# AIBluefisher/DReg-NeRF

Hardware: AMD Instinct MI355X
Metric: nerf_pairs_per_sec_regtr_fwd_bwd_128 (higher is better)
Workload: dtype bf16; 1 GPU; RegTR fwd+bwd+AdamW, shell-R synthetic pairs, 128^3 grids, 4 pairs (8 grids) per GPU per step, random-init weights; global_batch_pairs=4, resolution=128, fpn_head=active-set (identical results; rows around occupied voxels), parallelism=dp1

## Files before the change

### dreg_nerf_amd/csrc/common.h

```cpp
#pragma once
#include <hip/hip_runtime.h>
#include <stdint.h>

#define DREG_OK 0
#define DREG_EINVAL (-1)
#define DREG_ELAUNCH (-2)

typedef uint16_t bf16_t;
typedef __attribute__((ext_vector_type(8))) short bf16x8_t;
typedef __attribute__((ext_vector_type(4))) short bf16x4_t;
typedef __attribute__((ext_vector_type(4))) float f32x4_t;
typedef __attribute__((ext_vector_type(16))) float f32x16_t;

__device__ __forceinline__ float bf2f(bf16_t h) { return __uint_as_float(((uint32_t)h) << 16); }
typedef __attribute__((__vector_size__(2 * sizeof(__bf16)))) __bf16 hw_bf16x2_t;
typedef __attribute__((__vector_size__(2 * sizeof(float)))) float hw_f32x2_t;
__device__ __forceinline__ bf16_t f2bf(float f) { return __builtin_bit_cast(unsigned short, (__bf16)f); }
__device__ __forceinline__ uint32_t f2bf2(float lo, float hi) {
    const hw_f32x2_t v = {lo, hi};
    return __builtin_bit_cast(uint32_t, __builtin_convertvector(v, hw_bf16x2_t));
}

template <typename T> struct Elem;
template <> struct Elem<float> {
    static __device__ __forceinline__ float ld(const float* p) { return *p; }
    static __device__ __forceinline__ void st(float* p, float v) { *p = v; }
};
template <> struct Elem<bf16_t> {
    static __device__ __forceinline__ float ld(const bf16_t* p) { return bf2f(*p); }
    static __device__ __forceinline__ void st(bf16_t* p, float v) { *p = f2bf(v); }
};

__device__ __forceinline__ uint32_t fdiv(uint32_t n, uint32_t magic) {
    return magic ? __umulhi(n, magic) : n;
}
static inline uint32_t host_magic(uint32_t d) {
    return d <= 1 ? 0u : (uint32_t)((0x100000000ull + d - 1) / d);
}

__device__ __forceinline__ float wave_sum(float v) {
#pragma unroll
    for (int o = 32; o > 0; o >>= 1) v += __shfl_xor(v, o, 64);
    return v;
}
__device__ __forceinline__ float wave_max(float v) {
#pragma unroll
    for (int o = 32; o > 0; o >>= 1) v = fmaxf(v, __shfl_xor(v, o, 64));
    return v;
}

#ifdef DREG_PROBE
#define DREG_KNOB(type, name, value) static type name = value
#else
#define DREG_KNOB(type, name, value) static constexpr type name = value
#endif

#define DREG_LAUNCH_CHECK()                                   \
    do {                                                      \
        hipError_t e__ = hipGetLastError();                   \
        if (e__ != hipSuccess) return (int)e__;               \
    } while (0)
```

### dreg_nerf_amd/csrc/pointset.hip

```cpp
#include "common.h"
#include <cstring>
#include <rocprim/device/device_radix_sort.hpp>
#include <rocprim/device/device_scan.hpp>

__device__ __forceinline__ void ld4(const float* p, float (&v)[4]) { const float4 q = *reinterpret_cast<const float4*>(p); v[0] = q.x; v[1] = q.y; v[2] = q.z; v[3] = q.w; }
__device__ __forceinline__ void ld4(const bf16_t* p, float (&v)[4]) {
    const uint2 q = *reinterpret_cast<const uint2*>(p);
    v[0] = __uint_as_float(q.x << 16); v[1] = __uint_as_float(q.x & 0xffff0000u); v[2] = __uint_as_float(q.y << 16); v[3] = __uint_as_float(q.y & 0xffff0000u);
}
__device__ __forceinline__ void st4(float* p, const float (&v)[4]) { *reinterpret_cast<float4*>(p) = make_float4(v[0], v[1], v[2], v[3]); }
__device__ __forceinline__ void st4(bf16_t* p, const float (&v)[4]) { *reinterpret_cast<uint2*>(p) = make_uint2(f2bf2(v[0], v[1]), f2bf2(v[2], v[3])); }
template <typename TO>
__global__ __launch_bounds__(256) void layernorm_fwd_kernel(const float* __restrict__ x, const float* __restrict__ g, const float* __restrict__ b,
                                                            const float* __restrict__ pe, TO* __restrict__ y, float* __restrict__ stats, int N, float eps)
{
    const int row = blockIdx.x * 4 + (threadIdx.x >> 6), lane = threadIdx.x & 63;
    if (row >= N) return;
    const float4 v = *reinterpret_cast<const float4*>(x + (size_t)row * 256 + lane * 4);
    const float mean = wave_sum(v.x + v.y + v.z + v.w) * (1.f / 256.f);
    const float d0 = v.x - mean, d1 = v.y - mean, d2 = v.z - mean, d3 = v.w - mean;
    const float var = wave_sum(d0 * d0 + d1 * d1 + d2 * d2 + d3 * d3) * (1.f / 256.f);
    const float rstd = 1.0f / sqrtf(var + eps);
    const float4 gg = *reinterpret_cast<const float4*>(g + lane * 4), bb = *reinterpret_cast<const float4*>(b + lane * 4);
    float o[4] = {d0 * rstd * gg.x + bb.x, d1 * rstd * gg.y + bb.y, d2 * rstd * gg.z + bb.z, d3 * rstd * gg.w + bb.w};
    if (pe) { const float4 p = *reinterpret_cast<const float4*>(pe + (size_t)row * 256 + lane * 4); o[0] += p.x; o[1] += p.y; o[2] += p.z; o[3] += p.w; }
    st4(y + (size_t)row * 256 + lane * 4, o);
    if (lane == 0) { stats[2 * row] = mean; stats[2 * row + 1] = rstd; }
}
__global__ __launch_bounds__(256) void layernorm_fwd2_kernel(const float* __restrict__ x, const float* __restrict__ g, const float* __restrict__ b,
                                                             const float* __restrict__ pe, int pe_rows, float* __restrict__ y32, bf16_t* __restrict__ y16,
                                                             float* __restrict__ stats, int N, float eps)
{
    const int row = blockIdx.x * 4 + (threadIdx.x >> 6), lane = threadIdx.x & 63;
    if (row >= N) return;
    const float4 v = *reinterpret_cast<const float4*>(x + (size_t)row * 256 + lane * 4);
    const float mean = wave_sum(v.x + v.y + v.z + v.w) * (1.f / 256.f);
    const float d0 = v.x - mean, d1 = v.y - mean, d2 = v.z - mean, d3 = v.w - mean;
    const float var = wave_sum(d0 * d0 + d1 * d1 + d2 * d2 + d3 * d3) * (1.f / 256.f);
    const float rstd = 1.0f / sqrtf(var + eps);
    const float4 gg = *reinterpret_cast<const float4*>(g + lane * 4), bb = *reinterpret_cast<const float4*>(b + lane * 4);
    float o[4] = {d0 * rstd * gg.x + bb.x, d1 * rstd * gg.y + bb.y, d2 * rstd * gg.z + bb.z, d3 * rstd * gg.w + bb.w};
    if (y32) st4(y32 + (size_t)row * 256 + lane * 4, o);
    if (y16) {
        if (pe) { const float4 p = *reinterpret_cast<const float4*>(pe + (size_t)(row % pe_rows) * 256 + lane * 4); o[0] += p.x; o[1] += p.y; o[2] += p.z; o[3] += p.w; }
        st4(y16 + (size_t)row * 256 + lane * 4, o);
    }
    if (lane == 0) { stats[2 * row] = mean; stats[2 * row + 1] = rstd; }
}
template <typename TG>
__global__ __launch_bounds__(256) void layernorm_bwd_kernel(const float* __restrict__ x, const TG* __restrict__ dy, const float* __restrict__ g,
                                                            const float* __restrict__ stats, float* __restrict__ dx, float* __restrict__ part,
                                                            int N, int rows_per_block, const float* dx_add, const float* dx_add2 = nullptr,
                                                            bf16_t* __restrict__ dx_bf = nullptr, const bf16_t* __restrict__ dy2 = nullptr)
{
    const int wave = threadIdx.x >> 6, lane = threadIdx.x & 63;
    const float4 gg = *reinterpret_cast<const float4*>(g + lane * 4);
    float dg[4] = {0, 0, 0, 0}, db[4] = {0, 0, 0, 0};
    const int r0 = blockIdx.x * rows_per_block;
    const int rend = min(r0 + rows_per_block, N);
    const float gv[4] = {gg.x, gg.y, gg.z, gg.w};
    for (int rb = r0 + wave; rb < rend; rb += 16) {
        constexpr int U = 4;
        float4 v[U], old[U], old2[U];
        float d[U][4], mean[U], rstd[U];
#pragma unroll
        for (int u = 0; u < U; ++u) {
            const int row = rb + 4 * u;
            if (row < rend) {
                v[u] = *reinterpret_cast<const float4*>(x + (size_t)row * 256 + lane * 4);
                ld4(dy + (size_t)row * 256 + lane * 4, d[u]);
                if (dy2) { float e2[4]; ld4(dy2 + (size_t)row * 256 + lane * 4, e2); d[u][0] += e2[0]; d[u][1] += e2[1]; d[u][2] += e2[2]; d[u][3] += e2[3]; }
                mean[u] = stats[2 * row]; rstd[u] = stats[2 * row + 1];
                if (dx_add) old[u] = *reinterpret_cast<const float4*>(dx_add + (size_t)row * 256 + lane * 4);
                if (dx_add2) old2[u] = *reinterpret_cast<const float4*>(dx_add2 + (size_t)row * 256 + lane * 4);
            }
        }
#pragma unroll
        for (int u = 0; u < U; ++u) {
            const int row = rb + 4 * u;
            if (row < rend) {
                const float xh[4] = {(v[u].x - mean[u]) * rstd[u], (v[u].y - mean[u]) * rstd[u], (v[u].z - mean[u]) * rstd[u], (v[u].w - mean[u]) * rstd[u]};
                float s1 = 0.f, s2 = 0.f;
#pragma unroll
                for (int i = 0; i < 4; ++i) { s1 += d[u][i] * gv[i]; s2 += d[u][i] * gv[i] * xh[i]; dg[i] += d[u][i] * xh[i]; db[i] += d[u][i]; }
                s1 = wave_sum(s1) * (1.f / 256.f); s2 = wave_sum(s2) * (1.f / 256.f);
                float o[4];
#pragma unroll
                for (int i = 0; i < 4; ++i) o[i] = rstd[u] * (d[u][i] * gv[i] - s1 - xh[i] * s2);
                if (dx_add) { o[0] += old[u].x; o[1] += old[u].y; o[2] += old[u].z; o[3] += old[u].w; }
                if (dx_add2) { o[0] += old2[u].x; o[1] += old2[u].y; o[2] += old2[u].z; o[3] += old2[u].w; }
                *reinterpret_cast<float4*>(dx + (size_t)row * 256 + lane * 4) = make_float4(o[0], o[1], o[2], o[3]);
                if (dx_bf) st4(dx_bf + (size_t)row * 256 + lane * 4, o);
            }
        }
    }
    __shared__ float red[4][512];
#pragma unroll
    for (int i = 0; i < 4; ++i) { red[wave][lane * 4 + i] = dg[i]; red[wave][256 + lane * 4 + i] = db[i]; }
    __syncthreads();
    for (int c = threadIdx.x; c < 512; c += 256) part[(size_t)blockIdx.x * 512 + c] = red[0][c] + red[1][c] + red[2][c] + red[3][c];
}
__global__ void layernorm_bwd_final_kernel(const float* __restrict__ part, float* __restrict__ dg, float* __restrict__ db, int nblk, int accumulate)
{
    const int c = blockIdx.x * (blockDim.x >> 6) + (threadIdx.x >> 6), lane = threadIdx.x & 63;
    if (c >= 512) return;
    double s = 0.0;
#pragma unroll 8
    for (int k = lane; k < nblk; k += 64) s += part[(size_t)k * 512 + c];
#pragma unroll
    for (int o = 32; o > 0; o >>= 1) s += __shfl_xor(s, o, 64);
    if (lane == 0) {
        float* dst = c < 256 ? dg + c : db + (c - 256);
        *dst = accumulate ? *dst + (float)s : (float)s;
    }
}

struct LnFinalDesc { const float* part; float* dg; float* db; int nblk, accumulate; };
static_assert(sizeof(LnFinalDesc) == 32, "LayerNorm final record: 32 bytes");
__global__ void layernorm_bwd_final_batched_kernel(const LnFinalDesc* __restrict__ descs)
{
    const LnFinalDesc d = descs[blockIdx.x >> 7];
    const int c = (blockIdx.x & 127) * (blockDim.x >> 6) + (threadIdx.x >> 6), lane = threadIdx.x & 63;
    if (c >= 512) return;
    double s = 0.0;
#pragma unroll 8
    for (int k = lane; k < d.nblk; k += 64) s += d.part[(size_t)k * 512 + c];
#pragma unroll
    for (int o = 32; o > 0; o >>= 1) s += __shfl_xor(s, o, 64);
    if (lane == 0) {
        float* dst = c < 256 ? d.dg + c : d.db + (c - 256);
        *dst = d.accumulate ? *dst + (float)s : (float)s;
    }
}

__global__ void posenc_sine_kernel(const float* __restrict__ xyz, float* __restrict__ pe, int N, float scale2pi, float log_temp)
{
    const size_t total = (size_t)N * 256;
    for (size_t i = blockIdx.x * (size_t)blockDim.x + threadIdx.x; i < total; i += (size_t)gridDim.x * blockDim.x) {
        const int c = (int)(i & 255), n = (int)(i >> 8);
        float v = 0.f;
        if (c < 252) {
            const int coord = c / 84, f = c - coord * 84;
            const float dim_t = powf(expf(log_temp), (float)(2 * (f >> 1)) / 84.f);
            const float arg = (xyz[(size_t)n * 3 + coord] * scale2pi) / dim_t;
            v = (f & 1) ? cosf(arg) : sinf(arg);
        }
        pe[i] = v;
    }
}

__global__ __launch_bounds__(256) void overlap_fwd_kernel(const float* __restrict__ f, const float* __restrict__ w, const float* __restrict__ b,
                                                          float* __restrict__ s, int N)
{
    const int row = blockIdx.x * 4 + (threadIdx.x >> 6), lane = threadIdx.x & 63;
    if (row >= N) return;
    const float4 v = *reinterpret_cast<const float4*>(f + (size_t)row * 256 + lane * 4);
    const float4 ww = *reinterpret_cast<const float4*>(w + lane * 4);
    const float z = wave_sum(v.x * ww.x + v.y * ww.y + v.z * ww.z + v.w * ww.w) + b[0];
    if (lane == 0) s[row] = 1.f / (1.f + expf(-z));
}
__global__ __launch_bounds__(256) void overlap_bwd_kernel(const float* __restrict__ f, const float* __restrict__ w, const float* __restrict__ s,
                                                          const float* __restrict__ gy, float* __restrict__ df, float* __restrict__ part,
                                                          int N, int rows_per_block, const float* df_add = nullptr)
{
    const int wave = threadIdx.x >> 6, lane = threadIdx.x & 63;
    const float4 ww = *reinterpret_cast<const float4*>(w + lane * 4);
    float dw[4] = {0, 0, 0, 0}, dbias = 0.f;
    const int r0 = blockIdx.x * rows_per_block;
    for (int row = r0 + wave; row < min(r0 + rows_per_block, N); row += 4) {
        const float sv = s[row], dl = gy[row] * sv * (1.f - sv);
        const float4 v = *reinterpret_cast<const float4*>(f + (size_t)row * 256 + lane * 4);
        float4 o = make_float4(dl * ww.x, dl * ww.y, dl * ww.z, dl * ww.w);
        if (df_add) {
            const float4 p = *reinterpret_cast<const float4*>(df_add + (size_t)row * 256 + lane * 4);
            o.x = p.x + o.x; o.y = p.y + o.y; o.z = p.z + o.z; o.w = p.w + o.w;
        }
        *reinterpret_cast<float4*>(df + (size_t)row * 256 + lane * 4) = o;
        dw[0] += dl * v.x; dw[1] += dl * v.y; dw[2] += dl * v.z; dw[3] += dl * v.w;
        dbias += dl;
    }
    __shared__ float red[4][257];
#pragma unroll
    for (int i = 0; i < 4; ++i) red[wave][lane * 4 + i] = dw[i];
    if (lane == 0) red[wave][256] = dbias;
    __syncthreads();
    for (int c = threadIdx.x; c < 257; c += 256) part[(size_t)blockIdx.x * 257 + c] = red[0][c] + red[1][c] + red[2][c] + red[3][c];
}
__global__ void overlap_bwd_final_kernel(const float* __restrict__ part, float* __restrict__ dw, float* __restrict__ db, int nblk, int accumulate = 0)
{
    const int c = blockIdx.x * (blockDim.x >> 6) + (threadIdx.x >> 6), lane = threadIdx.x & 63;
    if (c >= 257) return;
    double s = 0.0;
    for (int k = lane; k < nblk; k += 64) s += part[(size_t)k * 257 + c];
#pragma unroll
    for (int o = 32; o > 0; o >>= 1) s += __shfl_xor(s, o, 64);
    if (lane == 0) { float* dst = c < 256 ? dw + c : db; *dst = accumulate ? *dst + (float)s : (float)s; }
}

template <typename TY, typename TG, typename TO>
__global__ void relu_bwd_kernel(const TY* __restrict__ y, const TG* __restrict__ g, TO* __restrict__ out, size_t n)
{
    for (size_t i = blockIdx.x * (size_t)blockDim.x + threadIdx.x; i < n; i += (size_t)gridDim.x * blockDim.x)
        Elem<TO>::st(out + i, Elem<TY>::ld(y + i) > 0.f ? Elem<TG>::ld(g + i) : 0.f);
}

__device__ void jacobi_eig3(double A[3][3], double V[3][3])
{
    for (int i = 0; i < 3; ++i) for (int j = 0; j < 3; ++j) V[i][j] = (i == j);
    for (int sweep = 0; sweep < 30; ++sweep) {
        const double off = fabs(A[0][1]) + fabs(A[0][2]) + fabs(A[1][2]);
        if (off < 1e-300) break;
        for (int p = 0; p < 2; ++p)
            for (int q = p + 1; q < 3; ++q) {
                if (fabs(A[p][q]) < 1e-300) continue;
                const double theta = (A[q][q] - A[p][p]) / (2.0 * A[p][q]);
                const double t = (theta >= 0 ? 1.0 : -1.0) / (fabs(theta) + sqrt(theta * theta + 1.0));
                const double c = 1.0 / sqrt(t * t + 1.0), s = t * c;
                for (int k = 0; k < 3; ++k) { const double akp = A[k][p], akq = A[k][q]; A[k][p] = c * akp - s * akq; A[k][q] = s * akp + c * akq; }
                for (int k = 0; k < 3; ++k) { const double apk = A[p][k], aqk = A[q][k]; A[p][k] = c * apk - s * aqk; A[q][k] = s * apk + c * aqk; }
                for (int k = 0; k < 3; ++k) { const double vkp = V[k][p], vkq = V[k][q]; V[k][p] = c * vkp - s * vkq; V[k][q] = s * vkp + c * vkq; }
            }
    }
}
struct KabschDense {
    const float* A; const float* Bp; const float* Wp;
    __device__ __forceinline__ float a(int i, int c) const { return A[i * 3 + c]; }
    __device__ __forceinline__ float b(int i, int c) const { return Bp[i * 3 + c]; }
    __device__ __forceinline__ float w(int i) const { return Wp[i]; }
};
struct KabschPair {
    const float* xyz; const float* corr; const float* ov; int s0, ns, t0;
    __device__ __forceinline__ float a(int i, int c) const { return i < ns ? xyz[(size_t)(s0 + i) * 3 + c] : corr[(size_t)(t0 + i - ns) * 3 + c]; }
    __device__ __forceinline__ float b(int i, int c) const { return i < ns ? corr[(size_t)(s0 + i) * 3 + c] : xyz[(size_t)(t0 + i - ns) * 3 + c]; }
    __device__ __forceinline__ float w(int i) const { return i < ns ? ov[s0 + i] : ov[t0 + i - ns]; }
};
template <typename Acc> __device__ void kabsch_body(const Acc& X, int N, float* __restrict__ o, float eps);
__global__ __launch_bounds__(256) void kabsch_kernel(const float* __restrict__ a, const float* __restrict__ b, const float* __restrict__ w,
                                                     float* __restrict__ out, int N, float eps)
{
    const int p = blockIdx.x;
    KabschDense X{a + (size_t)p * N * 3, b + (size_t)p * N * 3, w + (size_t)p * N};
    kabsch_body(X, N, out + (size_t)p * 12, eps);
}
__global__ __launch_bounds__(256) void kabsch_pairs_kernel(const float* __restrict__ xyz, const float* __restrict__ corr, const float* __restrict__ ov,
                                                           const int* __restrict__ probs, float* __restrict__ out, int L, int R, float eps)
{
    const int p = blockIdx.x / L, l = blockIdx.x % L;
    const int* pr = probs + p * 4;
    KabschPair X{xyz, corr + (size_t)l * R * 3, ov + (size_t)l * R, pr[0], pr[1], pr[2]};
    kabsch_body(X, pr[1] + pr[3], out + (size_t)blockIdx.x * 12, eps);
}
struct KabschSums { double sw, norm, ca[3], cb[3], H[3][3]; };
template <typename Acc> __device__ void kabsch_sums(const Acc& X, int N, float eps, KabschSums& S)
{
    const int t = threadIdx.x;
    __shared__ double red[9][256];
    __shared__ double tot[9];
    auto block_sums = [&](double* v, int NV) {
        for (int q = 0; q < NV; ++q) red[q][t] = v[q];
        __syncthreads();
        if (t < 64) {
            for (int q = 0; q < NV; ++q) {
                double a = (red[q][t] + red[q][t + 128]) + (red[q][t + 64] + red[q][t + 192]);
#pragma unroll
                for (int s = 32; s > 0; s >>= 1) a += __shfl_down(a, s, 64);
                if (t == 0) tot[q] = a;
            }
        }
        __syncthreads();
        for (int q = 0; q < NV; ++q) v[q] = tot[q];
        __syncthreads();
    };
    double sw = 0.0;
#pragma unroll 4
    for (int i = t; i < N; i += 256) sw += X.w(i);
    block_sums(&sw, 1);
    const double norm = fmax(sw, (double)eps);
    double ca[3] = {0, 0, 0}, cb[3] = {0, 0, 0};
#pragma unroll 2
    for (int i = t; i < N; i += 256) {
        const double wn = X.w(i) / norm;
        for (int c = 0; c < 3; ++c) { ca[c] += wn * X.a(i, c); cb[c] += wn * X.b(i, c); }
    }
    {
        double v6[6] = {ca[0], ca[1], ca[2], cb[0], cb[1], cb[2]};
        block_sums(v6, 6);
        for (int c = 0; c < 3; ++c) { ca[c] = v6[c]; cb[c] = v6[3 + c]; }
    }
    double H[3][3] = {{0, 0, 0}, {0, 0, 0}, {0, 0, 0}};
#pragma unroll 2
    for (int i = t; i < N; i += 256) {
        const double wn = X.w(i) / norm;
        for (int r = 0; r < 3; ++r) for (int c = 0; c < 3; ++c) H[r][c] += (X.a(i, r) - ca[r]) * (X.b(i, c) - cb[c]) * wn;
    }
    block_sums(&H[0][0], 9);
    S.sw = sw;
    S.norm = norm;
    for (int c = 0; c < 3; ++c) { S.ca[c] = ca[c]; S.cb[c] = cb[c]; }
    for (int r = 0; r < 3; ++r) for (int c = 0; c < 3; ++c) S.H[r][c] = H[r][c];
}
__device__ void kabsch_svd(const double (&H)[3][3], double (&U)[3][3], double (&Vs)[3][3])
{
    double HtH[3][3], V[3][3];
    for (int i = 0; i < 3; ++i) for (int j = 0; j < 3; ++j) { double s = 0; for (int k = 0; k < 3; ++k) s += H[k][i] * H[k][j]; HtH[i][j] = s; }
    jacobi_eig3(HtH, V);
    double ev[3] = {HtH[0][0], HtH[1][1], HtH[2][2]};
    int idx[3] = {0, 1, 2};
    for (int i = 0; i < 2; ++i) for (int j = i + 1; j < 3; ++j) if (ev[idx[j]] > ev[idx[i]]) { int tmp = idx[i]; idx[i] = idx[j]; idx[j] = tmp; }
    for (int k = 0; k < 3; ++k) for (int j = 0; j < 3; ++j) Vs[k][j] = V[k][idx[j]];
    for (int j = 0; j < 2; ++j) {
        double n2 = 0;
        for (int i = 0; i < 3; ++i) { double s = 0; for (int k = 0; k < 3; ++k) s += H[i][k] * Vs[k][j]; U[i][j] = s; n2 += s * s; }
        const double n = sqrt(n2);
        for (int i = 0; i < 3; ++i) U[i][j] = n > 0 ? U[i][j] / n : (i == j);
    }
    U[0][2] = U[1][0] * U[2][1] - U[2][0] * U[1][1]; U[1][2] = U[2][0] * U[0][1] - U[0][0] * U[2][1]; U[2][2] = U[0][0] * U[1][1] - U[1][0] * U[0][1];
    Vs[0][2] = Vs[1][0] * Vs[2][1] - Vs[2][0] * Vs[1][1]; Vs[1][2] = Vs[2][0] * Vs[0][1] - Vs[0][0] * Vs[2][1]; Vs[2][2] = Vs[0][0] * Vs[1][1] - Vs[1][0] * Vs[0][1];
}
__device__ __forceinline__ void kabsch_rotation(const double (&U)[3][3], const double (&V)[3][3], double (&R)[3][3])
{
    for (int i = 0; i < 3; ++i) for (int j = 0; j < 3; ++j) R[i][j] = V[i][0] * U[j][0] + V[i][1] * U[j][1] + V[i][2] * U[j][2];
}
template <typename Acc> __device__ void kabsch_body(const Acc& X, int N, float* __restrict__ o, float eps)
{
    KabschSums S;
    kabsch_sums(X, N, eps, S);
    if (threadIdx.x == 0) {
        double U[3][3], V[3][3], R[3][3];
        kabsch_svd(S.H, U, V);
        kabsch_rotation(U, V, R);
        for (int i = 0; i < 3; ++i) {
            double tr = S.cb[i];
            for (int j = 0; j < 3; ++j) { o[i * 4 + j] = (float)R[i][j]; tr -= R[i][j] * S.ca[j]; }
            o[i * 4 + 3] = (float)tr;
        }
    }
}

constexpr double KABSCH_BWD_GUARD = 1e-6;
struct KabschDenseGrad {
    float* ga; float* gb; float* gw;
    __device__ __forceinline__ void put(int i, const double (&a)[3], const double (&b)[3], double w) const {
        if (ga) for (int c = 0; c < 3; ++c) ga[i * 3 + c] = (float)a[c];
        if (gb) for (int c = 0; c < 3; ++c) gb[i * 3 + c] = (float)b[c];
        if (gw) gw[i] = (float)w;
    }
};
struct KabschPairGrad {
    float* gcorr; float* gov; int s0, ns, t0;
    __device__ __forceinline__ void put(int i, const double (&a)[3], const double (&b)[3], double w) const {
        const size_t r = i < ns ? (size_t)(s0 + i) : (size_t)(t0 + i - ns);
        const double* g = i < ns ? b : a;
        if (gcorr) for (int c = 0; c < 3; ++c) gcorr[r * 3 + c] = (float)g[c];
        if (gov) gov[r] = (float)w;
    }
};
template <typename Acc, typename Out> __device__ void kabsch_bwd_body(const Acc& X, int N, const float* __restrict__ g, float eps, const Out& Y)
{
    const int t = threadIdx.x;
    KabschSums S;
    kabsch_sums(X, N, eps, S);
    __shared__ double pub[16];
    if (t == 0) {
        double U[3][3], V[3][3], R[3][3];
        kabsch_svd(S.H, U, V);
        kabsch_rotation(U, V, R);
        double sig[3];
        for (int k = 0; k < 3; ++k) {
            double s = 0;
            for (int i = 0; i < 3; ++i) for (int j = 0; j < 3; ++j) s += U[i][k] * S.H[i][j] * V[j][k];
            sig[k] = s;
        }
        double G[3][3], gca[3], gcb[3];
        for (int i = 0; i < 3; ++i) {
            gcb[i] = g[i * 4 + 3];
            for (int j = 0; j < 3; ++j) G[i][j] = g[i * 4 + j] - g[i * 4 + 3] * S.ca[j];
        }
        for (int i = 0; i < 3; ++i) gca[i] = -(R[0][i] * gcb[0] + R[1][i] * gcb[1] + R[2][i] * gcb[2]);
        double GU[3][3], Gh[3][3], Yh[3][3], YV[3][3], Gb[3][3];
        for (int i = 0; i < 3; ++i) for (int j = 0; j < 3; ++j) GU[i][j] = G[i][0] * U[0][j] + G[i][1] * U[1][j] + G[i][2] * U[2][j];
        for (int i = 0; i < 3; ++i) for (int j = 0; j < 3; ++j) Gh[i][j] = V[0][i] * GU[0][j] + V[1][i] * GU[1][j] + V[2][i] * GU[2][j];
        const double tau = KABSCH_BWD_GUARD * sig[0];
        for (int i = 0; i < 3; ++i)
            for (int j = 0; j < 3; ++j) {
                const double d = sig[i] + sig[j];
                Yh[i][j] = (i == j || !(fabs(d) > tau)) ? 0.0 : (Gh[i][j] - Gh[j][i]) / d;
            }
        for (int i = 0; i < 3; ++i) for (int j = 0; j < 3; ++j) YV[i][j] = Yh[i][0] * V[j][0] + Yh[i][1] * V[j][1] + Yh[i][2] * V[j][2];
        for (int i = 0; i < 3; ++i) for (int j = 0; j < 3; ++j) Gb[i][j] = -(U[i][0] * YV[0][j] + U[i][1] * YV[1][j] + U[i][2] * YV[2][j]);
        const bool clamped = !(S.sw >= (double)eps);
        const double m = clamped ? S.sw / S.norm - 1.0 : 0.0;
// ... 649 lines not shown
```

### dreg_nerf_amd/csrc/pointset_exec.hip

```cpp
#include <hip/hip_runtime.h>
#include <cstdint>
#include <cstring>
#include <algorithm>
#include <vector>
#include "../../include/dreg_nerf.h"
#ifndef DREG_ELAUNCH
#define DREG_ELAUNCH (-2)
#endif

namespace {

constexpr int E = 256, E3 = 768, FF = 1024, NL = 6, NH = 8;
enum { N1W, N1B, SIW, SIB, SOW, SOB, N2W, N2B, CIW, CIB, COW, COB, N3W, N3B, L1W, L1B, L2W, L2B, PL_COUNT };
enum { FNW = NL * PL_COUNT, FNB, QW, QB, KW, KB, CW, CB, PS_NPARAM };
enum { LIN_SI, LIN_SO, LIN_CI, LIN_CO, LIN_1, LIN_2, LIN_PER_LAYER };
constexpr int NLIN = NL * LIN_PER_LAYER + 2;

struct Lin { int cout, cin, w, b; };
struct ReduceRec { const float* part; float* dw; int nsplit, Cout, Kpad, ntaps, Cin, Cin_real, accumulate, block0; };
static_assert(sizeof(ReduceRec) == 48, "matches WgradReduceDesc of conv.hip");
struct ColsumRec { const void* g; float* out; float* partial; int M, C, rpc, nch, pblock0, fblock0, accumulate, pad; };
static_assert(sizeof(ColsumRec) == 56, "matches ColsumDesc of fpn_ops.hip");
struct LnRec { const float* part; float* dg; float* db; int nblk, accumulate; };
static_assert(sizeof(LnRec) == 32, "matches LnFinalDesc of pointset.hip");

inline size_t al(size_t v) { return (v + 255) / 256 * 256; }

struct LayerBuf {
    size_t xa, xb, st1, st2, st3, h1, h2, h3, qkv1, qkv2, o1, o2, lse1, lse2, f;
    size_t gF, gB, gQ2, gC, gQ1;
    size_t wg[LIN_PER_LAYER], cs[LIN_PER_LAYER], lnp[3];
};
struct Layout {
    int R = -1;
    size_t allx, stf, dec_in, q, k, corr_lse;
    LayerBuf L[NL];
    size_t dallx, dallx_bf, dq, dk, ddec, ddec2, dH, dO, dvec, gx[2], lnpf[2], wgq, wgk, csq, csk, ov_ws, ks_ws, cs_ws, tables;
    size_t ks_bytes = 0, total = 0;
    size_t wg_bytes[NLIN];
};

struct Ps {
    float* val[PS_NPARAM];
    float* grad[PS_NPARAM];
    Lin lin[NLIN];
    Layout lay;
    int fuse = 1;
    int group_wgrad = 1;
    std::vector<hipEvent_t> ev;
    hipEvent_t ev_done = nullptr;
    static constexpr int RING = 8;
    static constexpr size_t TABLE_BYTES = 16384;
    char* pinned = nullptr;
    hipEvent_t ring_ev[RING] = {};
    unsigned ring_next = 0;
    struct Timed { hipEvent_t e0, e1; int kind, rows, cin, cout, flags; };
    bool timing = false;
    std::vector<Timed> timed;
    size_t timed_used = 0;
};

struct PsScope {
    Ps::Timed* t = nullptr; hipStream_t st;
    PsScope(Ps* p, void* stream, int kind, int rows, int cin, int cout, int flags) : st((hipStream_t)stream) {
        if (!p->timing) return;
        if (p->timed_used == p->timed.size()) {
            Ps::Timed n{};
            if (hipEventCreate(&n.e0) != hipSuccess || hipEventCreate(&n.e1) != hipSuccess) return;
            p->timed.push_back(n);
        }
        t = &p->timed[p->timed_used++];
        t->kind = kind; t->rows = rows; t->cin = cin; t->cout = cout; t->flags = flags;
        (void)hipEventRecord(t->e0, st);
    }
    ~PsScope() { if (t) (void)hipEventRecord(t->e1, st); }
};

inline int lin_index(int layer, int which) { return layer * LIN_PER_LAYER + which; }

void build_layout(Ps* p, int R)
{
    Layout& y = p->lay;
    if (y.R == R) return;
    y = Layout();
    y.R = R;
    size_t off = 0;
    auto take = [&](size_t bytes) { const size_t o = off; off += al(bytes); return o; };
    const size_t r = (size_t)R;
    y.allx = take(NL * r * E * 4);
    y.stf = take(NL * r * 2 * 4);
    y.dec_in = take(NL * r * E * 2);
    y.q = take(NL * r * E * 2);
    y.k = take(NL * r * E * 2);
    y.corr_lse = take(NL * r * 4);
    for (int i = 0; i < NLIN; ++i) {
        const Lin& l = p->lin[i];
        const int rows = i < NL * LIN_PER_LAYER ? R : NL * R;
        y.wg_bytes[i] = dreg_conv3d_wgrad_workspace_bytes(rows, 1, 1, 1, l.cin, l.cout, 1, 0);
        const size_t k1 = dreg_conv3d_igemm_workspace_bytes(rows, 1, 1, 1, l.cin, 1, 1, 1, l.cout, 1, 1, 0, 0, 0, 0);
        const size_t k2 = dreg_conv3d_igemm_workspace_bytes(rows, 1, 1, 1, l.cout, 1, 1, 1, l.cin, 1, 1, 0, 1, 0, 0);
        if (k1 > y.ks_bytes) y.ks_bytes = k1;
        if (k2 > y.ks_bytes) y.ks_bytes = k2;
    }
    const size_t lnp = dreg_layernorm_bwd_workspace_bytes(R), lnpf = dreg_layernorm_bwd_workspace_bytes(NL * R);
    for (int l = 0; l < NL; ++l) {
        LayerBuf& b = y.L[l];
        b.xa = take(r * E * 4); b.xb = take(r * E * 4);
        b.st1 = take(r * 8); b.st2 = take(r * 8); b.st3 = take(r * 8);
        b.h1 = take(r * E * 2); b.h2 = take(r * E * 2); b.h3 = take(r * E * 2);
        b.qkv1 = take(r * E3 * 2); b.qkv2 = take(r * E3 * 2);
        b.o1 = take(r * E * 2); b.o2 = take(r * E * 2);
        b.lse1 = take(NH * r * 4); b.lse2 = take(NH * r * 4);
        b.f = take(r * FF * 2);
        b.gF = take(r * FF * 2); b.gB = take(r * E * 2); b.gQ2 = take(r * E3 * 2); b.gC = take(r * E * 2); b.gQ1 = take(r * E3 * 2);
        for (int w = 0; w < LIN_PER_LAYER; ++w) {
            b.wg[w] = take(y.wg_bytes[lin_index(l, w)]);
            b.cs[w] = take(dreg_colsum_workspace_bytes(r, p->lin[lin_index(l, w)].cout));
        }
        for (int k = 0; k < 3; ++k) b.lnp[k] = take(lnp);
    }
    y.dallx = take(NL * r * E * 4);
    y.dallx_bf = take(NL * r * E * 2);
    y.dq = take(NL * r * E * 2); y.dk = take(NL * r * E * 2);
    y.ddec = take(NL * r * E * 2); y.ddec2 = take(NL * r * E * 2);
    y.dH = take(r * E * 2); y.dO = take(r * FF * 2);
    y.dvec = take((size_t)NL * r * 4 > NH * r * 4 ? NL * r * 4 : NH * r * 4);
    y.gx[0] = take(r * E * 4); y.gx[1] = take(r * E * 4);
    y.lnpf[0] = take(lnpf); y.lnpf[1] = take(lnpf);
    y.wgq = take(y.wg_bytes[NLIN - 2]); y.wgk = take(y.wg_bytes[NLIN - 1]);
    y.csq = take(dreg_colsum_workspace_bytes(NL * r, E)); y.csk = take(dreg_colsum_workspace_bytes(NL * r, E));
    y.ov_ws = take(dreg_overlap_bwd_workspace_bytes(NL * R));
    y.ks_ws = take(y.ks_bytes);
    y.cs_ws = take(dreg_colsum_workspace_bytes(NL * r, FF));
    y.tables = take(Ps::TABLE_BYTES);
    y.total = off + 256;
}

#define CK(expr) do { int rc_ = (expr); if (rc_) return rc_; } while (0)

int linear_fwd(Ps* p, const Layout& y, char* A, const void* x, const void* wpk, const float* bias, const void* residual, void* out,
               int rows, int cin, int cout, int relu, int out_f32, void* st)
{
    PsScope sc(p, st, 0, rows, cin, cout, (residual ? 1 : 0) | (out_f32 ? 2 : 0) | (y.ks_bytes ? 4 : 0));
    return dreg_conv3d_igemm_ws(x, wpk, out, bias, residual, rows, 1, 1, 1, cin, 1, 1, 1, cout, 1, 1, 0, 0, relu, residual ? 1 : 0, residual ? 1 : 0,
                                residual ? 1 : 0, residual ? 1 : 0, 0, out_f32, y.ks_bytes ? A + y.ks_ws : nullptr, y.ks_bytes, st);
}
int linear_dgrad(Ps* p, const Layout& y, char* A, const void* g, const void* wpk_t, void* gx, const void* mask, const void* add,
                 int rows, int cin, int cout, void* st)
{
    const void* addend = mask ? mask : add;
    PsScope sc(p, st, 1, rows, cin, cout, (addend ? 1 : 0) | (y.ks_bytes ? 4 : 0));
    return dreg_conv3d_igemm_ws(g, wpk_t, gx, nullptr, addend, rows, 1, 1, 1, cout, 1, 1, 1, cin, 1, 1, 0, 1, mask ? 2 : 0, addend ? 1 : 0, addend ? 1 : 0,
                                addend ? 1 : 0, addend ? 1 : 0, 0, 0, y.ks_bytes ? A + y.ks_ws : nullptr, y.ks_bytes, st);
}

}

extern "C" {

int dreg_ps_num_params(void) { return PS_NPARAM; }
int dreg_ps_num_linears(void) { return NLIN; }

void* dreg_ps_create(const int64_t* params)
{
    Ps* p = new Ps();
    for (int i = 0; i < PS_NPARAM; ++i) { p->val[i] = (float*)params[2 * i]; p->grad[i] = (float*)params[2 * i + 1]; }
    for (int l = 0; l < NL; ++l) {
        const int o = l * PL_COUNT;
        p->lin[lin_index(l, LIN_SI)] = {E3, E, o + SIW, o + SIB};
        p->lin[lin_index(l, LIN_SO)] = {E, E, o + SOW, o + SOB};
        p->lin[lin_index(l, LIN_CI)] = {E3, E, o + CIW, o + CIB};
        p->lin[lin_index(l, LIN_CO)] = {E, E, o + COW, o + COB};
        p->lin[lin_index(l, LIN_1)] = {FF, E, o + L1W, o + L1B};
        p->lin[lin_index(l, LIN_2)] = {E, FF, o + L2W, o + L2B};
    }
    p->lin[NLIN - 2] = {E, E, QW, QB};
    p->lin[NLIN - 1] = {E, E, KW, KB};
    if (hipHostMalloc((void**)&p->pinned, Ps::RING * Ps::TABLE_BYTES, hipHostMallocDefault) != hipSuccess) { delete p; return nullptr; }
    return p;
}
void dreg_ps_destroy(void* h)
{
    Ps* p = (Ps*)h;
    if (!p) return;
    for (auto& e : p->ev) if (e) (void)hipEventDestroy(e);
    if (p->ev_done) (void)hipEventDestroy(p->ev_done);
    for (auto& e : p->ring_ev) if (e) (void)hipEventDestroy(e);
    for (auto& t : p->timed) { (void)hipEventDestroy(t.e0); (void)hipEventDestroy(t.e1); }
    if (p->pinned) (void)hipHostFree(p->pinned);
    delete p;
}
void dreg_ps_set_fuse(void* h, int fuse) { ((Ps*)h)->fuse = fuse ? 1 : 0; }
void dreg_ps_set_group_wgrad(void* h, int on) { ((Ps*)h)->group_wgrad = on ? 1 : 0; }
void dreg_ps_set_timing(void* h, int enable) { ((Ps*)h)->timing = enable != 0; }
int dreg_ps_read_timings(void* h, int* info, float* ms, int cap)
{
    Ps* p = (Ps*)h;
    int n = 0;
    for (size_t i = 0; i < p->timed_used && n < cap; ++i) {
        const Ps::Timed& t = p->timed[i];
        float v = 0.f;
        if (hipEventElapsedTime(&v, t.e0, t.e1) != hipSuccess) continue;
        info[5 * n] = t.kind; info[5 * n + 1] = t.rows; info[5 * n + 2] = t.cin; info[5 * n + 3] = t.cout; info[5 * n + 4] = t.flags;
        ms[n++] = v;
    }
    p->timed_used = 0;
    return n;
}
size_t dreg_ps_arena_bytes(void* h, int R) { Ps* p = (Ps*)h; build_layout(p, R); return p->lay.total; }

int dreg_ps_forward(void* h, void* arena, size_t arena_bytes, const int64_t* packs, const float* feats, const float* xyz, const float* pe,
                    const int* probs_self, const int* probs_cross, int nprob, int max_len, int R,
                    float* cond, float* corr, float* ov, void* stream)
{
    Ps* p = (Ps*)h;
    if (R <= 0) return DREG_EINVAL;
    build_layout(p, R);
    const Layout& y = p->lay;
    if (arena_bytes < y.total) return DREG_EINVAL;
    char* A = (char*)arena;
    const float sc = 0.17677669529663687f;
    auto pk = [&](int li, int t) { return (const void*)packs[2 * li + t]; };
    const float* xin = feats;
    for (int l = 0; l < NL; ++l) {
        const LayerBuf& b = y.L[l];
        const int o = l * PL_COUNT;
        float* xout = (float*)(A + y.allx) + (size_t)l * R * E;
        CK(dreg_layernorm_fwd(xin, p->val[o + N1W], p->val[o + N1B], pe, A + b.h1, (float*)(A + b.st1), R, E, 1e-5f, 0, stream));
        CK(linear_fwd(p, y, A, A + b.h1, pk(lin_index(l, LIN_SI), 0), p->val[o + SIB], nullptr, A + b.qkv1, R, E, E3, 0, 0, stream));
        CK(dreg_mha_varlen_fwd(A + b.qkv1, A + b.qkv1 + E * 2, A + b.qkv1 + 2 * E * 2, A + b.o1, (float*)(A + b.lse1), probs_self, nprob, max_len, max_len,
                               R, NH, E3, E3, E3, E, sc, 0, stream));
        CK(linear_fwd(p, y, A, A + b.o1, pk(lin_index(l, LIN_SO), 0), p->val[o + SOB], xin, A + b.xa, R, E, E, 0, 1, stream));
        CK(dreg_layernorm_fwd((const float*)(A + b.xa), p->val[o + N2W], p->val[o + N2B], pe, A + b.h2, (float*)(A + b.st2), R, E, 1e-5f, 0, stream));
        CK(linear_fwd(p, y, A, A + b.h2, pk(lin_index(l, LIN_CI), 0), p->val[o + CIB], nullptr, A + b.qkv2, R, E, E3, 0, 0, stream));
        CK(dreg_mha_varlen_fwd(A + b.qkv2, A + b.qkv2 + E * 2, A + b.qkv2 + 2 * E * 2, A + b.o2, (float*)(A + b.lse2), probs_cross, nprob, max_len, max_len,
                               R, NH, E3, E3, E3, E, sc, 0, stream));
        CK(linear_fwd(p, y, A, A + b.o2, pk(lin_index(l, LIN_CO), 0), p->val[o + COB], A + b.xa, A + b.xb, R, E, E, 0, 1, stream));
        CK(dreg_layernorm_fwd((const float*)(A + b.xb), p->val[o + N3W], p->val[o + N3B], nullptr, A + b.h3, (float*)(A + b.st3), R, E, 1e-5f, 0, stream));
        CK(linear_fwd(p, y, A, A + b.h3, pk(lin_index(l, LIN_1), 0), p->val[o + L1B], nullptr, A + b.f, R, E, FF, 1, 0, stream));
        CK(linear_fwd(p, y, A, A + b.f, pk(lin_index(l, LIN_2), 0), p->val[o + L2B], A + b.xb, xout, R, FF, E, 0, 1, stream));
        xin = xout;
    }
    const int R6 = NL * R;
    CK(dreg_layernorm_fwd2((const float*)(A + y.allx), p->val[FNW], p->val[FNB], pe, R, cond, A + y.dec_in, (float*)(A + y.stf), R6, E, 1e-5f, stream));
    CK(linear_fwd(p, y, A, A + y.dec_in, pk(NLIN - 2, 0), p->val[QB], nullptr, A + y.q, R6, E, E, 0, 0, stream));
    CK(linear_fwd(p, y, A, A + y.dec_in, pk(NLIN - 1, 0), p->val[KB], nullptr, A + y.k, R6, E, E, 0, 0, stream));
    CK(dreg_corr_attention_varlen_fwd(A + y.q, A + y.k, xyz, corr, (float*)(A + y.corr_lse), probs_cross, nprob, max_len, max_len, NL, R, 0.0625f, 0, stream));
    CK(dreg_overlap_fwd(cond, p->val[CW], p->val[CB], ov, R6, stream));
    return DREG_OK;
}

int dreg_ps_backward(void* h, void* arena, size_t arena_bytes, const int64_t* packs, const float* feats, const float* xyz, const float* pe,
                     const int* probs_self, const int* probs_cross, int nprob, int max_len, int R,
                     const float* cond, const float* corr, const float* ov, const float* g_cond, const float* g_corr, const float* g_ov,
                     float* d_feats, void* stream, void* aux_stream, int last_only)
{
    Ps* p = (Ps*)h;
    if (R <= 0 || R != p->lay.R) return DREG_EINVAL;
    const Layout& y = p->lay;
    if (arena_bytes < y.total) return DREG_EINVAL;
    for (int i = 0; i < PS_NPARAM; ++i) if (!p->grad[i]) return DREG_EINVAL;
    char* A = (char*)arena;
    hipStream_t st = (hipStream_t)stream;
    hipStream_t ax = aux_stream && aux_stream != stream ? (hipStream_t)aux_stream : st;
    const bool two = ax != st;
    const float sc = 0.17677669529663687f;
    const int LB = last_only ? NL - 1 : 0, nlb = last_only ? 1 : NL;
    const int R6 = nlb * R;
    const size_t rb = (size_t)LB * R;
    const int fuse = p->fuse;
    auto pk = [&](int li, int t) { return (const void*)packs[2 * li + t]; };
    cond += rb * E; corr += rb * 3; ov += rb;
    if (p->ev.size() < (size_t)NLIN + 2) {
        p->ev.resize(NLIN + 2, nullptr);
        for (auto& e : p->ev) if (!e && hipEventCreateWithFlags(&e, hipEventDisableTiming) != hipSuccess) return DREG_ELAUNCH;
        if (hipEventCreateWithFlags(&p->ev_done, hipEventDisableTiming) != hipSuccess) return DREG_ELAUNCH;
    }
    std::vector<ReduceRec> rd;
    std::vector<ColsumRec> cs;
    std::vector<LnRec> ln;
    int rd_blocks = 0, cs_p = 0, cs_f = 0;
    struct GroupRec { char d[160]; int variant, nblocks; };
    std::vector<GroupRec> grp;
    const bool group = fuse && p->group_wgrad && !p->timing;
    auto param_grads = [&](int li, const void* g, const void* x, int rows, size_t wg_off, size_t cs_off) -> int {
        const Lin& l = p->lin[li];
        bool grouped = false;
        if (group) {
            GroupRec gr{};
            if (dreg_linear_wgrad_group_fill(gr.d, g, x, A + wg_off, y.wg_bytes[li], rows, l.cin, l.cout, &gr.variant, &gr.nblocks) == DREG_OK) { grp.push_back(gr); grouped = true; }
        }
        if (!grouped) {
            if (two) { if (hipEventRecord(p->ev[li], st) != hipSuccess || hipStreamWaitEvent(ax, p->ev[li], 0) != hipSuccess) return DREG_ELAUNCH; }
            PsScope sc(p, ax, 2, rows, l.cin, l.cout, 0);
            CK(dreg_conv3d_wgrad_partials(g, x, A + wg_off, y.wg_bytes[li], nullptr, 0, rows, 1, 1, 1, l.cin, l.cin, 1, 1, 1, l.cout, 1, 1, 0, nullptr, ax));
        }
        ReduceRec r{};
        r.part = (const float*)(A + wg_off); r.dw = p->grad[l.w];
        r.nsplit = dreg_conv3d_wgrad_splits(rows, 1, 1, 1, l.cin, l.cout, 1, 0);
        r.Cout = l.cout; r.Kpad = dreg_conv3d_kpad(1, l.cin, 0); r.ntaps = 1; r.Cin = l.cin; r.Cin_real = l.cin; r.accumulate = 1; r.block0 = rd_blocks;
        rd_blocks += dreg_wgrad_reduce_blocks(l.cout, l.cin, 1, r.nsplit);
        rd.push_back(r);
        if (!fuse) return dreg_colsum(g, p->grad[l.b], (float*)(A + y.cs_ws), (size_t)rows, l.cout, 1, 0, ax);
        ColsumRec c{};
        c.g = g; c.out = p->grad[l.b]; c.partial = (float*)(A + cs_off); c.M = rows; c.C = l.cout;
        c.rpc = dreg_colsum_rows_per_chunk((size_t)rows); c.nch = (rows + c.rpc - 1) / c.rpc; c.pblock0 = cs_p; c.fblock0 = cs_f; c.accumulate = 1;
        cs_p += c.nch; cs_f += (l.cout + 3) / 4;
        cs.push_back(c);
        return DREG_OK;
    };
    auto ln_rec = [&](size_t part_off, int wi, int bi, int rows) {
        LnRec r{(const float*)(A + part_off), p->grad[wi], p->grad[bi], dreg_layernorm_bwd_blocks(rows), 1};
        ln.push_back(r);
    };

    const float* Gcond = g_cond;
    if (g_ov) {
        CK(dreg_overlap_bwd_acc(cond, p->val[CW], ov, g_ov, (float*)(A + y.dallx) + rb * E, g_cond, p->grad[CW], p->grad[CB], 1, (float*)(A + y.ov_ws), R6, stream));
        Gcond = (const float*)(A + y.dallx) + rb * E;
    }
    bool have_dec = false;
    if (g_corr) {
        const size_t ob = rb * E * 2;
        CK(dreg_corr_attention_varlen_bwd(A + y.q + ob, A + y.k + ob, xyz, corr, g_corr, (const float*)(A + y.corr_lse) + rb, (float*)(A + y.dvec), A + y.dq + ob, A + y.dk + ob,
                                          probs_cross, nprob, max_len, max_len, nlb, R, 0.0625f, 0, stream));
        CK(param_grads(NLIN - 1, A + y.dk + ob, A + y.dec_in + ob, R6, y.wgk, y.csk));
        CK(param_grads(NLIN - 2, A + y.dq + ob, A + y.dec_in + ob, R6, y.wgq, y.csq));
        CK(linear_dgrad(p, y, A, A + y.dk + ob, pk(NLIN - 1, 1), A + y.ddec + ob, nullptr, nullptr, R6, E, E, stream));
        if (fuse) CK(linear_dgrad(p, y, A, A + y.dq + ob, pk(NLIN - 2, 1), A + y.ddec + ob, nullptr, A + y.ddec + ob, R6, E, E, stream));
        else {
            CK(linear_dgrad(p, y, A, A + y.dq + ob, pk(NLIN - 2, 1), A + y.ddec2 + ob, nullptr, nullptr, R6, E, E, stream));
            CK(dreg_add_inplace(A + y.ddec + ob, A + y.ddec2 + ob, (size_t)R6 * E, 0, stream));
        }
        have_dec = true;
    }
    float* dallx = (float*)(A + y.dallx);
    const float* allx = (const float*)(A + y.allx);
    {
        const float* ax = allx + rb * E;
        const float* stf = (const float*)(A + y.stf) + rb * 2;
        float* dg = dallx + rb * E;
        char* dgb = A + y.dallx_bf + rb * E * 2;
        const char* dd = A + y.ddec + rb * E * 2;
    if (Gcond && have_dec && fuse) {
        CK(dreg_layernorm_bwd_parts(ax, Gcond, dd, p->val[FNW], stf, dg, nullptr, nullptr, dgb, (float*)(A + y.lnpf[0]), R6, E, 1, stream));
        ln_rec(y.lnpf[0], FNW, FNB, R6);
    } else if (Gcond || have_dec) {
        bool first = true;
        if (Gcond) {
            CK(dreg_layernorm_bwd_parts(ax, Gcond, nullptr, p->val[FNW], stf, dg, nullptr, nullptr, have_dec ? nullptr : dgb, (float*)(A + y.lnpf[0]), R6, E, 1, stream));
            ln_rec(y.lnpf[0], FNW, FNB, R6);
            first = false;
        }
        if (have_dec) {
            CK(dreg_layernorm_bwd_parts(ax, dd, nullptr, p->val[FNW], stf, dg, first ? nullptr : dg, nullptr, dgb, (float*)(A + y.lnpf[1]), R6, E, 0, stream));
            ln_rec(y.lnpf[1], FNW, FNB, R6);
        }
    } else {
        return DREG_EINVAL;
    }
    }

    const float* G = dallx + (size_t)(NL - 1) * R * E;
    const void* Gbf = A + y.dallx_bf + (size_t)(NL - 1) * R * E * 2;
    for (int l = NL - 1; l >= 0; --l) {
        const LayerBuf& b = y.L[l];
        const int o = l * PL_COUNT;
        const float* xin = l == 0 ? feats : allx + (size_t)(l - 1) * R * E;
        if (fuse) CK(linear_dgrad(p, y, A, Gbf, pk(lin_index(l, LIN_2), 1), A + b.gF, A + b.f, nullptr, R, FF, E, stream));
        else {
            CK(linear_dgrad(p, y, A, Gbf, pk(lin_index(l, LIN_2), 1), A + y.dO, nullptr, nullptr, R, FF, E, stream));
            CK(dreg_relu_bwd(A + b.f, A + y.dO, A + b.gF, (size_t)R * FF, 0, 0, 0, stream));
        }
        CK(param_grads(lin_index(l, LIN_2), Gbf, A + b.f, R, b.wg[LIN_2], b.cs[LIN_2]));
        CK(linear_dgrad(p, y, A, A + b.gF, pk(lin_index(l, LIN_1), 1), A + y.dH, nullptr, nullptr, R, E, FF, stream));
        CK(param_grads(lin_index(l, LIN_1), A + b.gF, A + b.h3, R, b.wg[LIN_1], b.cs[LIN_1]));
        float* Gb = (float*)(A + y.gx[0]);
        CK(dreg_layernorm_bwd_parts((const float*)(A + b.xb), A + y.dH, nullptr, p->val[o + N3W], (const float*)(A + b.st3), Gb, G, nullptr, A + b.gB,
                                    (float*)(A + b.lnp[2]), R, E, 0, stream));
        ln_rec(b.lnp[2], o + N3W, o + N3B, R);
        CK(linear_dgrad(p, y, A, A + b.gB, pk(lin_index(l, LIN_CO), 1), A + y.dO, nullptr, nullptr, R, E, E, stream));
        CK(param_grads(lin_index(l, LIN_CO), A + b.gB, A + b.o2, R, b.wg[LIN_CO], b.cs[LIN_CO]));
        CK(dreg_mha_varlen_bwd(A + b.qkv2, A + b.qkv2 + E * 2, A + b.qkv2 + 2 * E * 2, A + b.o2, A + y.dO, (const float*)(A + b.lse2), (float*)(A + y.dvec),
                               A + b.gQ2, A + b.gQ2 + E * 2, A + b.gQ2 + 2 * E * 2, probs_cross, nprob, max_len, max_len, R, NH, E3, E3, E3, E, sc, 0, stream));
        CK(linear_dgrad(p, y, A, A + b.gQ2, pk(lin_index(l, LIN_CI), 1), A + y.dH, nullptr, nullptr, R, E, E3, stream));
        CK(param_grads(lin_index(l, LIN_CI), A + b.gQ2, A + b.h2, R, b.wg[LIN_CI], b.cs[LIN_CI]));
        float* Ga = (float*)(A + y.gx[1]);
        CK(dreg_layernorm_bwd_parts((const float*)(A + b.xa), A + y.dH, nullptr, p->val[o + N2W], (const float*)(A + b.st2), Ga, Gb, nullptr, A + b.gC,
                                    (float*)(A + b.lnp[1]), R, E, 0, stream));
        ln_rec(b.lnp[1], o + N2W, o + N2B, R);
        CK(linear_dgrad(p, y, A, A + b.gC, pk(lin_index(l, LIN_SO), 1), A + y.dO, nullptr, nullptr, R, E, E, stream));
        CK(param_grads(lin_index(l, LIN_SO), A + b.gC, A + b.o1, R, b.wg[LIN_SO], b.cs[LIN_SO]));
        CK(dreg_mha_varlen_bwd(A + b.qkv1, A + b.qkv1 + E * 2, A + b.qkv1 + 2 * E * 2, A + b.o1, A + y.dO, (const float*)(A + b.lse1), (float*)(A + y.dvec),
                               A + b.gQ1, A + b.gQ1 + E * 2, A + b.gQ1 + 2 * E * 2, probs_self, nprob, max_len, max_len, R, NH, E3, E3, E3, E, sc, 0, stream));
        CK(linear_dgrad(p, y, A, A + b.gQ1, pk(lin_index(l, LIN_SI), 1), A + y.dH, nullptr, nullptr, R, E, E3, stream));
        CK(param_grads(lin_index(l, LIN_SI), A + b.gQ1, A + b.h1, R, b.wg[LIN_SI], b.cs[LIN_SI]));
        if (l == 0) {
            CK(dreg_layernorm_bwd_parts(xin, A + y.dH, nullptr, p->val[o + N1W], (const float*)(A + b.st1), d_feats, Ga, nullptr, nullptr,
                                        (float*)(A + b.lnp[0]), R, E, 0, stream));
        } else {
            float* Gprev = dallx + (size_t)(l - 1) * R * E;
            void* Gprev_bf = A + y.dallx_bf + (size_t)(l - 1) * R * E * 2;
            CK(dreg_layernorm_bwd_parts(xin, A + y.dH, nullptr, p->val[o + N1W], (const float*)(A + b.st1), Gprev, Ga, last_only ? nullptr : Gprev, Gprev_bf,
                                        (float*)(A + b.lnp[0]), R, E, 0, stream));
            G = Gprev; Gbf = Gprev_bf;
        }
        ln_rec(b.lnp[0], o + N1W, o + N1B, R);
    }

    const size_t nb_rd = rd.size() * sizeof(ReduceRec), nb_cs = cs.size() * sizeof(ColsumRec), nb_ln = ln.size() * sizeof(LnRec);
    const size_t o_cs = al(nb_rd), o_ln = o_cs + al(nb_cs);
    const int gd = dreg_wgrad_group_desc_bytes();
    std::stable_sort(grp.begin(), grp.end(), [](const GroupRec& a, const GroupRec& b) { return a.variant < b.variant; });
    const size_t o_grp = al(o_ln + nb_ln), nb_grp = grp.size() * (size_t)gd;
    if (gd > 160 || o_grp + nb_grp > Ps::TABLE_BYTES) return DREG_EINVAL;
    if (o_ln + nb_ln > Ps::TABLE_BYTES) return DREG_EINVAL;
    const unsigned slot = p->ring_next++ % Ps::RING;
    if (!p->ring_ev[slot]) { if (hipEventCreateWithFlags(&p->ring_ev[slot], hipEventDisableTiming) != hipSuccess) return DREG_ELAUNCH; }
    else if (hipEventSynchronize(p->ring_ev[slot]) != hipSuccess) return DREG_ELAUNCH;
    char* host = p->pinned + (size_t)slot * Ps::TABLE_BYTES;
    std::memcpy(host, rd.data(), nb_rd);
    std::memcpy(host + o_cs, cs.data(), nb_cs);
    std::memcpy(host + o_ln, ln.data(), nb_ln);
    struct GroupLaunch { size_t off; int n, variant, blocks; };
    std::vector<GroupLaunch> gl;
    for (size_t i = 0; i < grp.size(); ++i) {
        if (gl.empty() || gl.back().variant != grp[i].variant) gl.push_back(GroupLaunch{o_grp + i * (size_t)gd, 0, grp[i].variant, 0});
        const int b0 = gl.back().blocks;
        std::memcpy(grp[i].d + gd - (int)sizeof(int), &b0, sizeof(int));
        std::memcpy(host + o_grp + i * (size_t)gd, grp[i].d, (size_t)gd);
        gl.back().n += 1; gl.back().blocks += grp[i].nblocks;
    }
    if (hipMemcpyAsync(A + y.tables, host, grp.empty() ? o_ln + nb_ln : o_grp + nb_grp, hipMemcpyHostToDevice, st) != hipSuccess) return DREG_ELAUNCH;
    if (hipEventRecord(p->ring_ev[slot], st) != hipSuccess) return DREG_ELAUNCH;
    if (two && hipStreamWaitEvent(ax, p->ring_ev[slot], 0) != hipSuccess) return DREG_ELAUNCH;
    const int ln_dup = (ln.size() >= 2 && ln[0].dg == ln[1].dg) ? 1 : 0;
    if (ln_dup) CK(dreg_layernorm_bwd_final_batched(A + y.tables + o_ln, 1, stream));
    CK(dreg_layernorm_bwd_final_batched(A + y.tables + o_ln + ln_dup * sizeof(LnRec), (int)ln.size() - ln_dup, stream));
    for (const GroupLaunch& q : gl) CK(dreg_wgrad_group_launch(A + y.tables + q.off, q.n, q.variant, q.blocks, ax));
    CK(dreg_wgrad_reduce_batched(A + y.tables, (int)rd.size(), 0, rd_blocks, ax));
    if (fuse) CK(dreg_colsum_batched(A + y.tables + o_cs, (int)cs.size(), cs_p, cs_f, ax));
    return DREG_OK;
}

}
```

### dreg_nerf_amd/lib.py

```python
import ctypes
import os
from ctypes import c_float, c_int, c_size_t, c_void_p

import torch

_HERE = os.path.dirname(os.path.abspath(__file__))
LIB_PATH = os.path.join(_HERE, "libdreg_nerf_hip.so")

DT_BF16 = 0
DT_F32 = 1

_lib = None


class DregError(RuntimeError):
    pass


def _sig(lib, name, restype, argtypes):
    fn = getattr(lib, name)
    fn.restype = restype
    fn.argtypes = argtypes
    return fn


P, I, F, Z = c_void_p, c_int, c_float, c_size_t

SIGNATURES = {
    "dreg_conv3d_igemm": (I, [P, P, P, P, P] + [I] * 18 + [I, I, P]),
    "dreg_conv3d_igemm_workspace_bytes": (Z, [I] * 15),
    "dreg_conv3d_igemm_ws": (I, [P, P, P, P, P] + [I] * 18 + [I, I, P, Z, P]),
    "dreg_conv3d_igemm_occ": (I, [P, P, P, P, P] + [I] * 18 + [I, I, P, Z, P, P]),
    "dreg_conv3d_igemm_bnstats": (I, [P, P, P, P, P] + [I] * 17 + [P, Z, P, P, P]),
    "dreg_conv3d_kpad": (I, [I, I, I]),
    "dreg_gemm_f32_desc_bytes": (I, []),
    "dreg_gemm_f32_batched": (I, [P, I, I, P, P]),
    "dreg_infonce_wsym": (I, [P, P, I, P]),
    "dreg_conv3d_igemm_defer": (I, [P, P, P, P, P] + [I] * 18 + [P, Z, P, P, P, P]),
    "dreg_bn3d_fwd_ex": (I, [P] * 10 + [I, I, I, F, F, I, I, I, P, P, I, P, P]),
    "dreg_bn3d_bwd_ex": (I, [P] * 11 + [I] * 6 + [P, P, P, P]),
    "dreg_exec_default_opts": (None, [P]),
    "dreg_exec_guard_bands": (I, [P]),
    "dreg_exec_guard_check": (I, [P, P, P, P]),
    "dreg_exec_guard_describe": (I, [P, I, P, I]),
    "dreg_exec_guard_last": (I, [P, P, P, P]),
    "dreg_guard_fill": (I, [P, P, I, I, P]),
    "dreg_guard_scan": (I, [P, P, I, I, P, P]),
    "dreg_exec_create_opts": (P, [P, I, P, I, P, I, P]),
    "dreg_ps_set_group_wgrad": (None, [P, I]),
    "dreg_conv_get_glds": (I, []),
    "dreg_conv3d_dgrad_s2": (I, [P, P, P] + [I] * 11 + [P]),
    "dreg_conv3d_dgrad_s2_acc": (I, [P, P, P] + [I] * 11 + [P]),
    "dreg_pack_conv_weight": (I, [P, P, I, I, I, I, I, I, P]),
    "dreg_pack_conv_weights_batched": (I, [P, I, I, I, P, P]),
    "dreg_conv3d_wgrad_splits": (I, [I] * 8),
    "dreg_conv3d_wgrad_workspace_bytes": (Z, [I] * 8),
    "dreg_conv3d_wgrad": (I, [P, P, P, P, Z] + [I] * 16 + [P]),
    "dreg_conv3d_wgrad_occ": (I, [P, P, P, P, Z] + [I] * 16 + [P, P]),
    "dreg_conv3d_igemm_rows": (I, [P] * 5 + [P, I] + [I] * 18 + [I, P]),
    "dreg_conv3d_wgrad_rows": (I, [P, P, P, P, Z] + [P, I] + [I] * 14 + [P]),
    "dreg_conv3d_wgrad_partials": (I, [P, P, P, Z, P, I] + [I] * 13 + [P, P]),
    "dreg_wgrad_reduce_blocks": (I, [I, I, I, I]),
    "dreg_wgrad_reduce_batched": (I, [P, I, I, I, P]),
    "dreg_conv3_halo_supported": (I, [I] * 6),
    "dreg_conv3_halo_use": (I, [I] * 9),
    "dreg_conv3_halo_pack_bytes": (Z, [I]),
    "dreg_pack_conv_weight_halo": (I, [P, P, I, I, I, P]),
    "dreg_conv3_halo": (I, [P, P, P, P, P] + [I] * 10 + [P]),
    "dreg_conv3_halo_pack_bytes_n": (Z, [I, I]),
    "dreg_conv3_halo_n": (I, [P, P, P, P, P] + [I] * 11 + [P]),
    "dreg_conv3_halo_n_bnstats": (I, [P, P, P, P, P] + [I] * 10 + [P, P, P]),
    "dreg_conv3d_wgrad_variant": (I, [I] * 10),
    "dreg_conv3d_igemm_variant": (I, [I] * 17),
    "dreg_conv3d_wgrad_group_fill": (I, [P, P, P, P, Z] + [I] * 12 + [P, P]),
    "dreg_bn_small_in_regs": (I, [I, I, I, I]),
    "dreg_wgrad_group_desc_bytes": (I, []),
    "dreg_linear_wgrad_group_fill": (I, [P, P, P, P, Z, I, I, I, P, P]),
    "dreg_wgrad_group_launch": (I, [P, I, I, I, P]),
    "dreg_bn_num_chunks": (I, [I]),
    "dreg_bn_relu_maxpool_fwd": (I, [P] * 10 + [I] * 8 + [F, F, I, I, P]),
    "dreg_bn_relu_maxpool_bwd": (I, [P] * 10 + [I] * 10 + [P]),
    "dreg_sparse_stem_workspace_floats": (Z, [I] * 5),
    "dreg_sparse_stem_fwd": (I, [P, P, I, P, I] + [P] * 12 + [I] * 8 + [F, F, I, I, P]),
    "dreg_sparse_stem_bwd": (I, [P] * 6 + [I, P, I] + [P] * 7 + [I] * 10 + [P]),
    "dreg_bn3d_fwd": (I, [P] * 10 + [I, I, I, F, F, I, I, I, P]),
    "dreg_bn3d_bwd": (I, [P] * 11 + [I, I, I, I, I, I, P]),
    "dreg_bn_small": (I, [I, I, I, I]),
    "dreg_bn3d_fwd_defer_update": (I, [P] * 10 + [I, I, I, F, F, I, I, I, P, P, P]),
    "dreg_bn3d_fwd_from_sums": (I, [P] * 10 + [I, I, I, I, F, F, I, I, P]),
    "dreg_bn3d_bwd_defer_params": (I, [P] * 11 + [I, I, I, I, I, I, P, P, P]),
    "dreg_bn_running_update_batched": (I, [P, I, I, I, F, P]),
    "dreg_bn_param_grad_batched": (I, [P, I, I, I, I, P]),
    "dreg_maxpool3d_fwd": (I, [P, P, P] + [I] * 9 + [P]),
    "dreg_maxpool3d_bwd": (I, [P, P, P] + [I] * 9 + [P]),
    "dreg_maxpool3d_bwd_acc": (I, [P, P, P] + [I] * 10 + [P]),
    "dreg_downsample_sum": (I, [P, P] + [I] * 9 + [P]),
    "dreg_downsample_sum_rows": (I, [P, P, P] + [I] * 9 + [P]),
    "dreg_colsum_workspace_bytes": (Z, [Z, I]),
    "dreg_colsum": (I, [P, P, P, Z, I, I, I, P]),
    "dreg_trilinear_gather_fwd": (I, [P, P, P, P] + [I] * 10 + [P]),
    "dreg_trilinear_gather_bwd": (I, [P, P, P, P] + [I] * 8 + [P]),
    "dreg_cast_from_f32": (I, [P, P, Z, I, P]),
    "dreg_fill_zero": (I, [P, Z, P]),
    "dreg_active_sets_workspace_bytes": (Z, [I] * 4),
    "dreg_active_sets": (I, [P, P] + [I] * 8 + [P, P, P, P, Z, P]),
    "dreg_active_sets_level2_workspace_bytes": (Z, [I] * 4),
    "dreg_active_sets_level2": (I, [P] + [I] * 7 + [P, P, P, Z, P]),
    "dreg_conv_rows_workspace_bytes": (Z, [I, I, I, I]),
    "dreg_conv_rows": (I, [P, P, I, I, I, I, I, I, I, I, I, I, I, P, P, P, Z, P]),
    "dreg_trilinear_gather_bwd_rows": (I, [P, P, P, P, I, P, P, P] + [I] * 10 + [P]),
    "dreg_colsum_rows": (I, [P, P, I, P, P, I, I, I, P]),
    "dreg_trilinear_gather_bwd_gather": (I, [P, P, P, P, I, P, P] + [I] * 10 + [P]),
    "dreg_trilinear_gather_bwd_gather_rows_only": (I, [P, P, P, P, I, P, P] + [I] * 10 + [P]),
    "dreg_trilinear_gather_bwd_gather_seg": (I, [P, P, P, P, P, I, P, P] + [I] * 11 + [P]),
    "dreg_gather_segment_mean": (I, [P, P, P, I, P, P, P, P] + [I] * 9 + [P]),
    "dreg_zero_rows": (I, [P, P, I, I, I, P]),
    "dreg_add_inplace": (I, [P, P, Z, I, P]),
    "dreg_pack_rgba_grids": (I, [P, P, I, I, I, I, I, P]),
    "dreg_pack_rgba_grids_occ": (I, [P, P, P, I, I, I, I, I, P]),
    "dreg_pack_rgba_sparse": (I, [P, P, P, P, I, I, I, I, I, I, P]),
    "dreg_pack_rgba_sparse_occ": (I, [P, P, P, P, P, I, I, I, I, I, I, P]),
    "dreg_conv_row_occupancy": (I, [P, P, I, I, I, I, I, I, I, I, P]),
    "dreg_gather_grid_xyz": (I, [P, P, P, P, I, I, I, I, P]),
    "dreg_exec_create": (P, [P, I, P, I, P, I]),
    "dreg_exec_destroy": (None, [P]),
    "dreg_exec_op_halo": (I, [P, I]),
    "dreg_exec_arena_bytes": (Z, [P]),
    "dreg_exec_pack_bytes": (Z, [P]),
    "dreg_exec_num_packs": (I, [P]),
    "dreg_exec_tensor_offset": (Z, [P, I]),
    "dreg_exec_output_slot": (I, [P]),
    "dreg_exec_pack_rows": (I, [P]),
    "dreg_exec_export_pack_table": (I, [P, P, P, P]),
    "dreg_exec_repack": (I, [P, P, P, P]),
    "dreg_exec_set_overlap": (None, [P, I]),
    "dreg_exec_set_input_row_occupancy": (None, [P, P]),
    "dreg_exec_set_timing": (None, [P, I]),
    "dreg_exec_read_timings": (I, [P, P, P, I]),
    "dreg_exec_forward": (I, [P, P, Z, P, P, P, I, I, P]),
    "dreg_exec_backward": (I, [P, P, Z, P, P, P, P, I, P, P]),
    "dreg_exec_backward_range": (I, [P, P, Z, P, P, P, P, I, P, P, I, I, I]),
    "dreg_mha_fwd": (I, [P] * 5 + [I] * 7 + [F, I, P]),
    "dreg_mha_bwd": (I, [P] * 10 + [I] * 7 + [F, I, P]),
    "dreg_corr_attention_fwd": (I, [P] * 5 + [I] * 3 + [F, I, P]),
    "dreg_corr_attention_bwd": (I, [P] * 9 + [I] * 3 + [F, I, P]),
    "dreg_mha_varlen_fwd": (I, [P] * 6 + [I] * 9 + [F, I, P]),
    "dreg_mha_varlen_bwd": (I, [P] * 11 + [I] * 9 + [F, I, P]),
    "dreg_corr_attention_varlen_fwd": (I, [P] * 6 + [I] * 5 + [F, I, P]),
    "dreg_corr_attention_varlen_bwd": (I, [P] * 10 + [I] * 5 + [F, I, P]),
    "dreg_layernorm_fwd": (I, [P] * 6 + [I, I, F, I, P]),
    "dreg_layernorm_bwd_workspace_bytes": (Z, [I]),
    "dreg_layernorm_bwd": (I, [P] * 8 + [I] * 5 + [P]),
    "dreg_layernorm_bwd_add": (I, [P] * 9 + [I] * 4 + [P]),
    "dreg_layernorm_fwd2": (I, [P, P, P, P, I, P, P, P, I, I, F, P]),
    "dreg_layernorm_bwd_parts": (I, [P] * 10 + [I, I, I, P]),
    "dreg_layernorm_bwd_blocks": (I, [I]),
    "dreg_layernorm_bwd_final_batched": (I, [P, I, P]),
    "dreg_overlap_bwd_acc": (I, [P, P, P, P, P, P, P, P, I, P, I, P]),
    "dreg_colsum_rows_per_chunk": (I, [Z]),
    "dreg_colsum_batched": (I, [P, I, I, I, P]),
    "dreg_brick_supported": (I, [I] * 6),
    "dreg_conv3_brick_pack_bytes": (Z, [I, I]),
    "dreg_pack_conv_weight_brick": (I, [P, P, I, I, I, P]),
    "dreg_brick_tiles_workspace_bytes": (Z, [I] * 4),
    "dreg_brick_tiles_build": (I, [P, I, I, I, I, I, I, P, Z, P, P, P, P, P, P]),
    "dreg_conv3_brick": (I, [P, P, P, P, P, P, I, P, P, P] + [I] * 11 + [P]),
    "dreg_ps_num_params": (I, []),
    "dreg_ps_num_linears": (I, []),
    "dreg_ps_create": (P, [P]),
    "dreg_ps_destroy": (None, [P]),
    "dreg_ps_set_fuse": (None, [P, I]),
    "dreg_ps_set_timing": (None, [P, I]),
    "dreg_ps_read_timings": (I, [P, P, P, I]),
    "dreg_ps_arena_bytes": (Z, [P, I]),
    "dreg_ps_forward": (I, [P, P, Z, P, P, P, P, P, P, I, I, I, P, P, P, P]),
    "dreg_ps_backward": (I, [P, P, Z, P, P, P, P, P, P, I, I, I, P, P, P, P, P, P, P, P, P, I]),
    "dreg_posenc_sine": (I, [P, P, I, F, F, P]),
    "dreg_overlap_fwd": (I, [P, P, P, P, I, P]),
    "dreg_overlap_bwd_workspace_bytes": (Z, [I]),
    "dreg_overlap_bwd": (I, [P] * 8 + [I, P]),
    "dreg_relu_bwd": (I, [P, P, P, Z, I, I, I, P]),
    "dreg_weighted_kabsch": (I, [P, P, P, P, I, I, F, P]),
    "dreg_weighted_kabsch_pairs": (I, [P, P, P, P, P, I, I, I, F, P]),
    "dreg_weighted_kabsch_bwd": (I, [P] * 7 + [I, I, F, P]),
    "dreg_weighted_kabsch_pairs_bwd": (I, [P] * 7 + [I, I, I, F, P]),
    "dreg_reg_point_losses": (I, [P] * 10 + [I, I, I, I, F, F, F, P]),
    "dreg_infonce_nn": (I, [P] * 7 + [I, I, F, P]),
    "dreg_infonce_rows": (I, [P] * 10 + [I, I, F, F, I, P]),
    "dreg_reg_losses_final": (I, [P] * 6 + [I, I, F, F, F, F, F, P]),
    "dreg_nerf_cont_deferred": (I, [P] * 5 + [I, I, I, F, F, F, F, P]),
    "dreg_halfspace_labels": (I, [P, P, P, P, I, I, P]),
    "dreg_voxel_downsample_workspace_bytes": (Z, [I]),
    "dreg_voxel_downsample_fwd": (I, [P] * 11 + [Z, I, I, I, F, P]),
    "dreg_voxel_downsample_bwd": (I, [P, P, P, P, I, I, P]),
    "dreg_voxel_downsample_plan": (I, [P] * 11 + [Z, I, I, F, P]),
    "dreg_voxel_downsample_plan_frozen": (I, [P] * 11 + [Z, I, I, F, P, P]),
    "dreg_voxel_segment_mean": (I, [P] * 5 + [I, I, P]),
    "dreg_grad_norm": (I, [P, P, P, Z, P]),
    "dreg_adamw_step": (I, [P] * 5 + [Z] + [F] * 5 + [I, F, P]),
    "dreg_ngp_level_table": (ctypes.c_uint32, [F, I, I, P, P, P, P, P]),
    "dreg_f32_to_f16": (I, [P, P, Z, P]),
    "dreg_ngp_density_fwd": (I, [P] * 6 + [P] * 5 + [P, I, P]),
    "dreg_ngp_rgb_mean_fwd": (I, [P] * 6 + [I, I, P]),
    "dreg_ngp_dir_bias": (I, [P, P, P, I, P]),
    "dreg_ngp_alpha_keep": (I, [P, P, P, I, F, F, P]),
    "dreg_ngp_density_fwd_contract": (I, [P] * 6 + [P] * 5 + [P, I, I, P]),
    "dreg_ngp_density_fwd_ws": (I, [P] * 6 + [P] * 5 + [P, I, I, P, Z, P, I, P]),
    "dreg_grid_sample_points_ordered": (I, [P, P, P, P, P, I, I, I, P, I, P]),
    "dreg_grid_x_order_workspace_bytes": (Z, [I, I, I]),
    "dreg_grid_x_order": (I, [P, P, P, P, Z, I, I, I, I, P]),
    "dreg_grid_occupied_workspace_bytes": (Z, [I, I, I]),
    "dreg_grid_occupied_totals": (P, [P, I, I, I]),
    "dreg_grid_occupied_count": (I, [P, P, Z, I, I, I, P]),
    "dreg_grid_occupied_build": (I, [P, P, P, P, P, P, P, P, I, I, I, I, P]),
    "dreg_ngp_density_keep_fwd_ws": (I, [P] * 6 + [P] * 5 + [P, I, I, P, Z, P, I] + [P, P, F, F, P]),
    "dreg_grid_write_kept": (I, [P, P, P, P, P, P, P, P, I, I, I, I, P]),
    "dreg_ngp_density_workspace_bytes": (Z, [I]),
    "dreg_ngp_rgb_dir_fwd": (I, [P] * 6 + [I, P]),
    "dreg_grid_scatter7": (I, [P] * 6 + [I, P]),
    "dreg_grid_sample_points": (I, [P, P, P, I, I, I, P, I, P]),
    "dreg_surface_visibility": (I, [P] * 7 + [P] * 5 + [P, P, P] + [I] * 5 + [F, F, F, F, P]),
    "dreg_surface_visibility_queue": (I, [P] * 7 + [P] * 5 + [P, P, P] + [I] * 5 + [F, F, F, F, P, P, P]),
    "dreg_occupancy_coarse_bits": (I, [P, P, I, I, I, P]),
    "dreg_surface_visibility_desc_bytes": (Z, []),
    "dreg_surface_visibility_fill_desc": (I, [P] + [P] * 7 + [P] * 5 + [P, P, P] + [I] * 5 + [F, F, F, F, P, P]),
    "dreg_surface_visibility_multi": (I, [P, I, ctypes.c_long, P]),
    "dreg_surface_visibility_multi_waves": (I, [P, I, ctypes.c_long, I, P]),
    "dreg_ngp_render": (I, [P, P, ctypes.c_long, P, I, I, I, P] + [P] * 6 + [P] * 5 + [P, P, P] + [F] * 5 + [P] + [P] * 6),
    "dreg_ngp_render_pair": (I, [ctypes.c_long] + ([P, P, P, I, I, I, P] + [P] * 6 + [P] * 5 + [P, P, P] + [F] * 4 + [P]) * 2 + [F, F, P] + [P] * 7),
    "dreg_ngp_render_train": (I, [P, P, P, ctypes.c_long, P, I, I, I, P] + [P] * 6 + [P] * 5 + [P, P, P] + [F] * 5 + [P] + [P] * 6),
    "dreg_ngp_render_bwd_workspace_bytes": (Z, [ctypes.c_long]),
    "dreg_ngp_render_bwd": (I, [P, P, P, ctypes.c_long, P, I, I, I, P, P, P] + [P] * 5 + [P, P, P] + [F] * 5 + [P, P, P, P, P, Z, P]),
    "dreg_ngp_adam_step": (I, [P] * 5 + [Z, F, F, F, F, I, P]),
    "dreg_image_metrics_workspace_bytes": (Z, [I, I, I, I]),
    "dreg_image_metrics": (I, [P, P, I, I, I, I, P] + [P] * 6 + [P, Z, P]),
    "dreg_ngp_density_grad": (I, [P] * 7 + [P] * 5 + [P, I, I, P]),
    "dreg_icp_workspace_bytes": (Z, [I, I]),
    "dreg_icp_refine": (I, [P, I, P, P, P, P, I, P, F, I, I, I, P, F, I] + [ctypes.c_double] * 3 + [P, P, P, P, P, Z, P]),
    "dreg_pose_ransac_workspace_bytes": (Z, [I, I]),
    "dreg_pose_ransac": (I, [P, P, I, P, I, F, F, P, Z, P, P, P, P, P, P, P]),
    "dreg_pose_inliers": (I, [P, P, I, P, F, P, P, P]),
    "dreg_mc_table": (I, [P, P]),
    "dreg_mc_workspace_bytes": (Z, [I, I, I]),
    "dreg_mc_count": (I, [P, I, I, I, F, P, Z, P, P]),
    "dreg_mc_emit": (I, [P, I, I, I, F, P, P, P, Z, P, P, I, I, P]),
}


PROBE_SIGNATURES = {
    "dreg_conv1_bnrelu_a_probe": (I, [P, P, P, P, I, I, I, I, I, I, P]),
    "dreg_conv_set_glds": (None, [I]),
    "dreg_conv_set_wgrad_splits": (None, [I]),
    "dreg_conv_set_wgrad_big": (None, [I]),
    "dreg_conv_igemm_probe": (None, [I]),
    "dreg_conv_set_igemm_ap": (None, [I]),
    "dreg_conv_set_igemm_ap256": (None, [I]),
    "dreg_conv_set_pointwise_rmw_cin": (None, [I]),
    "dreg_conv_igemm_probe_read": (I, [P]),
    "dreg_conv_set_wgrad_pipe": (None, [I]),
    "dreg_conv_wgrad_probe_read": (I, [P]),
    "dreg_conv_set_wgrad_ring": (None, [I]),
    "dreg_conv_set_wgrad_rows_fast": (None, [I]),
    "dreg_conv_set_row_splits": (None, [I]),
    "dreg_conv_set_glds_stages": (None, [I]),
    "dreg_conv_set_wgrad_target_blocks": (None, [I]),
    "dreg_conv_set_narrow_small": (None, [I]),
    "dreg_bn_set_debug_skip": (None, [I]),
    "dreg_bn_set_store_g": (None, [I]),
    "dreg_bn_set_small_regs": (None, [I]),
    "dreg_sstem_set_pool_blocks": (None, [I]),
    "dreg_voxel_set_own_sort": (None, [I]),
    "dreg_conv_set_bn_stats_epilogue": (None, [I]),
    "dreg_conv3_halo_set_variant": (None, [I]),
    "dreg_conv3_halo64_set": (None, [I]),
    "dreg_conv3_halo_set_prof": (None, [P]),
    "dreg_bn_set_small_max_voxels": (None, [I]),
    "dreg_ngp_set_rgb_chunks": (None, [I]),
    "dreg_ngp_set_density_unroll": (None, [I]),
    "dreg_ngp_set_xcd_levels": (None, [I]),
    "dreg_visibility_set_waves": (None, [I]),
    "dreg_visibility_set_pass_bound": (I, [ctypes.c_long]),
    "dreg_render_set_waves": (None, [I]),
    "dreg_render_pair_set_waves": (None, [I]),
    "dreg_render_bwd_set_waves": (None, [I]),
}
PROBE_LIB_PATH = os.path.join(_HERE, "libdreg_nerf_hip_probe.so")
_probe_lib = None


class ExecOpts(ctypes.Structure):
    _fields_ = [(n, c_int) for n in ("sparse_grads", "bn_batch_tails", "fuse_stem", "sparse_stem", "fold_res_bn", "fold_splitk", "group_wgrad",
                                     "s2_accumulate", "fuse_bn_stats", "brick", "defer_head_pg", "persistent_deep", "guard")] + [("reserved", c_int * 3)]


def load_probe():
    global _probe_lib
    if _probe_lib is None:
        if not os.path.exists(PROBE_LIB_PATH):
            raise DregError(f"{PROBE_LIB_PATH} not found: build it with `python -m dreg_nerf_amd.build`")
        lib = ctypes.CDLL(PROBE_LIB_PATH)
        for name, (rt, at) in list(SIGNATURES.items()) + list(PROBE_SIGNATURES.items()):
            _sig(lib, name, rt, at)
        _probe_lib = lib
    return _probe_lib


def use_probe():
    global _lib
    _lib = load_probe()
    return _lib


class probe:

    def __init__(self):
        self._restore = []

    def __enter__(self):
        global _lib
        self._saved = _lib
        _lib = load_probe()
        self.lib = _lib
        return self

    def set(self, name, value, default):
        getattr(self.lib, name)(value)
        self._restore.append((name, default))

    def __getattr__(self, name):
        return getattr(self.__dict__["lib"], name)

    def __exit__(self, *exc):
        global _lib
        for name, default in reversed(self._restore):
            getattr(self.lib, name)(default)
        _lib = self._saved
        return False


def load():
    global _lib
    if _lib is None:
        if not os.path.exists(LIB_PATH):
            raise DregError(
                f"{LIB_PATH} not found: build it with `python -m dreg_nerf_amd.build` "
                "(hipcc --offload-arch=gfx950); dreg_nerf_amd has no CPU/eager fallback")
        lib = ctypes.CDLL(LIB_PATH)
        for name, (rt, at) in SIGNATURES.items():
            _sig(lib, name, rt, at)
        _lib = lib
    return _lib


def declared_symbols():
    return list(SIGNATURES.keys())


def probe_symbols():
    return list(PROBE_SIGNATURES.keys())


def ptr(t):
    if t is None:
        return None
    assert t.is_contiguous(), "non-contiguous tensor handed to the C ABI"
    return t.data_ptr()


_raw_stream = getattr(torch._C, "_cuda_getCurrentRawStream", None)


def stream():
    if _raw_stream is not None:
        return _raw_stream(torch.cuda.current_device())
    return torch.cuda.current_stream().cuda_stream


_DEBUG_SYNC = bool(int(os.environ.get("DREG_DEBUG_SYNC", "0")))


def check(rc, name):
    if rc != 0:
        raise DregError(f"{name} failed with code {rc}")
    if _DEBUG_SYNC:
        import sys
        print(f"[dreg] {name} launched", file=sys.stderr, flush=True)
        torch.cuda.synchronize()


def dt_of(t: torch.Tensor) -> int:
    if t.dtype == torch.bfloat16:
        return DT_BF16
    if t.dtype == torch.float32:
        return DT_F32
    raise DregError(f"unsupported dtype {t.dtype}")


def torch_dtype(dt: int):
    return torch.bfloat16 if dt == DT_BF16 else torch.float32


def to_device_async(data, dtype, device):
    t = torch.tensor(data, dtype=dtype)
    if device.type != "cuda":
        return t
    return t.pin_memory().to(device, non_blocking=True)
```

### dreg_nerf_amd/pointset_exec.py

```python
import ctypes
from typing import Dict, Optional

import numpy as np
import torch

from . import lib as L
from . import ops

N_LAYERS = 6
_PER_LAYER = ("norm1.weight", "norm1.bias", "self_attn.in_proj_weight", "self_attn.in_proj_bias", "self_attn.out_proj.weight",
              "self_attn.out_proj.bias", "norm2.weight", "norm2.bias", "cross_attn.in_proj_weight", "cross_attn.in_proj_bias",
              "cross_attn.out_proj.weight", "cross_attn.out_proj.bias", "norm3.weight", "norm3.bias", "linear1.weight", "linear1.bias",
              "linear2.weight", "linear2.bias")
_TAIL = ("transformer_encoder.norm.weight", "transformer_encoder.norm.bias", "correspondence_decoder.q_proj.weight",
         "correspondence_decoder.q_proj.bias", "correspondence_decoder.k_proj.weight", "correspondence_decoder.k_proj.bias",
         "correspondence_decoder.conf_logits_decoder.weight", "correspondence_decoder.conf_logits_decoder.bias")
_LINEARS = ("self_attn.in_proj_weight", "self_attn.out_proj.weight", "cross_attn.in_proj_weight", "cross_attn.out_proj.weight",
            "linear1.weight", "linear2.weight")

FUSE = True
GROUP_WGRAD = True


def param_names():
    names = [f"transformer_encoder.layers.{l}.{n}" for l in range(N_LAYERS) for n in _PER_LAYER]
    return names + list(_TAIL)


def linear_names():
    names = [f"transformer_encoder.layers.{l}.{n}" for l in range(N_LAYERS) for n in _LINEARS]
    return names + ["correspondence_decoder.q_proj.weight", "correspondence_decoder.k_proj.weight"]


class PointSetExecutor:

    def __init__(self, P: Dict[str, torch.Tensor], with_grad: bool):
        self.lib = L.load()
        names = param_names()
        assert len(names) == self.lib.dreg_ps_num_params()
        self.params = [P[n] for n in names]
        self.linears = [P[n] for n in linear_names()]
        assert len(self.linears) == self.lib.dreg_ps_num_linears()
        self.with_grad = with_grad
        tab = np.zeros((len(names), 2), dtype=np.int64)
        self._sig = []
        for i, t in enumerate(self.params):
            assert t.is_contiguous() and t.dtype == torch.float32, "the executor reads fp32 master parameters in place"
            g = t.grad if with_grad else None
            if with_grad and (g is None or not g.is_contiguous() or g.dtype != torch.float32):
                raise L.DregError("PointSetExecutor needs preallocated contiguous fp32 .grad buffers (FlatAdamW) on every parameter")
            tab[i, 0] = t.data_ptr()
            tab[i, 1] = g.data_ptr() if g is not None else 0
            self._sig.append((t.data_ptr(), int(tab[i, 1])))
        self.h = self.lib.dreg_ps_create(tab.ctypes.data)
        if not self.h:
            raise L.DregError("dreg_ps_create failed")
        self.lib.dreg_ps_set_fuse(self.h, int(FUSE))
        self.lib.dreg_ps_set_group_wgrad(self.h, int(GROUP_WGRAD))
        self._fuse = FUSE
        self._group = GROUP_WGRAD
        self.device = self.params[0].device
        self.arena = None
        self.arena_bytes = 0
        self._timing = False
        self._packs = (ctypes.c_int64 * (2 * len(self.linears)))()
        self._pack_stamp = None
        self._pack_keep = None

    def __del__(self):
        try:
            if getattr(self, "h", None):
                self.lib.dreg_ps_destroy(self.h)
                self.h = None
        except Exception:
            pass

    def still_valid(self) -> bool:
        for t, (vp, gp) in zip(self.params, self._sig):
            g = t.grad if self.with_grad else None
            if t.data_ptr() != vp or (g.data_ptr() if g is not None else 0) != gp:
                return False
        return True

    def _pack_table(self):
        stamp = (ops._weight_generation, sum(t._version for t in self.linears))
        if stamp != self._pack_stamp:
            keep = []
            for i, w in enumerate(self.linears):
                f = ops.packed_weight(w, w.shape[1], False, L.DT_BF16)
                d = ops.packed_weight(w, w.shape[1], True, L.DT_BF16)
                self._packs[2 * i], self._packs[2 * i + 1] = f.data_ptr(), d.data_ptr()
                keep += [f, d]
            self._pack_keep, self._pack_stamp = keep, stamp
        return ctypes.addressof(self._packs)

    def _arena_for(self, R: int):
        need = self.lib.dreg_ps_arena_bytes(self.h, R)
        if need > self.arena_bytes:
            self.arena = None
            self.arena_bytes = int(need * 1.25)
            self.arena = torch.empty(self.arena_bytes, dtype=torch.uint8, device=self.device)
        return self.arena

    def set_timing(self, on: bool):
        self._timing = bool(on)
        self.lib.dreg_ps_set_timing(self.h, int(on))

    def drain_timings(self, profiler: "ops.KernelTimer"):
        cap = 4096
        info = (ctypes.c_int * (5 * cap))()
        ms = (ctypes.c_float * cap)()
        n = self.lib.dreg_ps_read_timings(self.h, info, ms, cap)
        for i in range(n):
            kind, rows, cin, cout, flags = (info[5 * i + k] for k in range(5))
            fl = 2.0 * rows * cin * cout
            if kind == 2:
                name = ops.wgrad_kernel_name(self.lib, rows, 1, 1, 1, cin, cout, 1)
                label = f"wgrad B{rows} 1x1x1x{cin} g1x1x1x{cout} k1s1"
            elif kind == 1:
                name = ops.igemm_kernel_name(self.lib, rows, 1, 1, 1, cout, 1, 1, 1, cin, 1, 1, 0, 1, 0, bool(flags & 4), bool(flags & 1), L.DT_BF16, False)
                label = f"dgrad B{rows} 1x1x1x{cout}->1x1x1x{cin} k1s1"
            else:
                name = ops.igemm_kernel_name(self.lib, rows, 1, 1, 1, cin, 1, 1, 1, cout, 1, 1, 0, 0, 0, bool(flags & 4), bool(flags & 1), L.DT_BF16, bool(flags & 2))
                label = f"fwd B{rows} 1x1x1x{cin}->1x1x1x{cout} k1s1"
            profiler.add_measured(name, label, fl, ms[i])

    def forward(self, feats, xyz, pe, tab):
        if self._fuse != FUSE:
            self.lib.dreg_ps_set_fuse(self.h, int(FUSE))
            self._fuse = FUSE
        if self._group != GROUP_WGRAD:
            self.lib.dreg_ps_set_group_wgrad(self.h, int(GROUP_WGRAD))
            self._group = GROUP_WGRAD
        want = ops.PROFILER is not None and ops.PROFILER.enabled
        if want != self._timing:
            self.set_timing(want)
        ops.wait_packs()
        R = feats.shape[0]
        arena = self._arena_for(R)
        dev = feats.device
        cond = torch.empty(N_LAYERS, R, 256, dtype=torch.float32, device=dev)
        corr = torch.empty(N_LAYERS, R, 3, dtype=torch.float32, device=dev)
        ov = torch.empty(N_LAYERS, R, 1, dtype=torch.float32, device=dev)
        L.check(self.lib.dreg_ps_forward(self.h, L.ptr(arena), self.arena_bytes, self._pack_table(), L.ptr(feats), L.ptr(xyz), L.ptr(pe),
                                         L.ptr(tab.self_probs), L.ptr(tab.cross_probs), tab.nprob, tab.max_len, R,
                                         L.ptr(cond), L.ptr(corr), L.ptr(ov), L.stream()), "dreg_ps_forward")
        self.generation = getattr(self, "generation", 0) + 1
        return cond, corr, ov

    def backward(self, feats, xyz, pe, tab, cond, corr, ov, g_cond, g_corr, g_ov, last_only=False, generation=None):
        if generation is not None and generation != getattr(self, "generation", 0):
            raise L.DregError("PointSetExecutor.backward: the shared arena was overwritten by a later forward pass (two grad-mode forwards before a "
                              "backward: gradient accumulation over several forwards / retain_graph need one executor per live graph)")
        R = feats.shape[0]
        d_feats = torch.empty_like(feats)
        aux = None if self._timing else ops.PARAM_GRAD_STREAM
        if aux is not None:
            self.arena.record_stream(aux)
        L.check(self.lib.dreg_ps_backward(self.h, L.ptr(self.arena), self.arena_bytes, self._pack_table(), L.ptr(feats), L.ptr(xyz), L.ptr(pe),
                                          L.ptr(tab.self_probs), L.ptr(tab.cross_probs), tab.nprob, tab.max_len, R,
                                          L.ptr(cond), L.ptr(corr), L.ptr(ov), L.ptr(g_cond), L.ptr(g_corr), L.ptr(g_ov), L.ptr(d_feats),
                                          L.stream(), aux.cuda_stream if aux is not None else None, int(last_only)), "dreg_ps_backward")
        return d_feats


class _PointSetFn(torch.autograd.Function):

    @staticmethod
    def forward(ctx, feats, anchor, ex: PointSetExecutor, xyz, pe, tab):
        cond, corr, ov = ex.forward(feats, xyz, pe, tab)
        ctx.ex, ctx.tab, ctx.generation = ex, tab, ex.generation
        ctx.save_for_backward(feats, xyz, pe, cond, corr, ov)
        ctx.set_materialize_grads(False)
        return cond, corr, ov, cond[-1].clone(), corr[-1].clone(), ov[-1].clone()

    @staticmethod
    def backward(ctx, g_cond, g_corr, g_ov, g_cl, g_rl, g_ol):
        feats, xyz, pe, cond, corr, ov = ctx.saved_tensors
        f32 = lambda g: g.contiguous().float() if g is not None else None
        if FUSE and g_cond is None and g_corr is None and g_ov is None:
            d_feats = ctx.ex.backward(feats, xyz, pe, ctx.tab, cond, corr, ov, f32(g_cl), f32(g_rl), f32(g_ol), last_only=True, generation=ctx.generation)
            return d_feats, None, None, None, None, None
        full = []
        for g, gl, ref in ((g_cond, g_cl, cond), (g_corr, g_rl, corr), (g_ov, g_ol, ov)):
            if gl is not None:
                g = torch.zeros_like(ref) if g is None else g.contiguous().float().clone()
                g[-1] += gl.float()
            full.append(f32(g))
        d_feats = ctx.ex.backward(feats, xyz, pe, ctx.tab, cond, corr, ov, *full, generation=ctx.generation)
        return d_feats, None, None, None, None, None


def executor_for(model, P) -> Optional[PointSetExecutor]:
    if model.precision != "bf16" or model.pos_emb_type != "sine" or not getattr(model, "native_pointset", True):
        return None
    names = param_names()
    train = torch.is_grad_enabled() and any(P[n].requires_grad for n in names)
    if train and not all(P[n].requires_grad for n in names):
        return None
    if train and any(P[n].grad is None or not P[n].grad.is_contiguous() for n in names):
        return None
    cache = model.__dict__.setdefault("_ps_cache", {})
    ex = cache.get(train)
    if ex is not None and not ex.still_valid():
        ex = None
    if ex is None:
        ex = cache[train] = PointSetExecutor(P, train)
    return ex


def encode_decode(ex: PointSetExecutor, feats, xyz, pe, tab, anchor, with_last: bool = False):
    feats = feats.float().contiguous()
    out = _PointSetFn.apply(feats, anchor, ex, xyz.contiguous(), pe.contiguous(), tab)
    return out if with_last else out[:3]
```

### include/dreg_nerf.h

```cpp
#ifndef DREG_NERF_H
#define DREG_NERF_H
#include <stddef.h>
#include <stdint.h>

#ifdef __cplusplus
extern "C" {
#endif

#define DREG_OK 0
#define DREG_EINVAL (-1)

int dreg_conv_get_glds(void);


int dreg_conv3d_kpad(int ksz, int Cin, int dtype);

int dreg_pack_conv_weight(const float* w, void* out, int Cout, int Cin_real, int Cin, int ksz, int for_dgrad,
                          int dtype, void* stream);
int dreg_pack_conv_weights_batched(const void* descs, int n, int total_rows, int stage_floats, const int* row_desc,
                                   void* stream);

int dreg_conv3d_igemm(const void* in, const void* wt_packed, void* out, const float* bias, const void* addend,
                      int B, int Di, int Hi, int Wi, int Cin, int Do, int Ho, int Wo, int Cout,
                      int ksz, int stride, int pad, int transposed, int relu, int Da, int Ha, int Wa, int add_same,
// ... 170 lines not shown
int dreg_trilinear_gather_bwd_gather_rows_only(const float* dfeat, const int64_t* idx, const int* pt_batch, const int* rows1, int n1,
                                               int* fine_map, void* dp1, int N, int B, int d, int h, int w, int C, int Zr, int Xr, int Yr,
                                               int dtype, void* stream);
int dreg_trilinear_gather_bwd_gather_seg(const float* g1, const void* seg_descs, const int64_t* idx, const int* pt_batch, const int* rows1, int n1,
                                         int* fine_map, void* dp1, int N, int B, int d, int h, int w, int C, int Zr, int Xr, int Yr,
                                         int dtype, int zero_dense, void* stream);
int dreg_gather_segment_mean(const void* p1, const int64_t* idx, const int* pt_batch, int point_start, const uint32_t* order, const uint32_t* starts,
                             const int* n_out, float* out, int M, int d, int h, int w, int C, int Zr, int Xr, int Yr, int dtype, void* stream);
int dreg_zero_rows(void* buf, const int* rows, int nrows, int C, int dtype, void* stream);
int dreg_colsum_rows(const void* g, const int* rows, int nrows, float* out, float* workspace, int C, int accumulate,
                     int dtype, void* stream);

void* dreg_exec_create(const int* tensors, int nt, const int* ops, int nops, const int64_t* params, int np);
typedef struct dreg_exec_opts {
    int sparse_grads;
    int bn_batch_tails;
    int fuse_stem;
    int sparse_stem;
    int fold_res_bn;
    int fold_splitk;
    int group_wgrad;
    int s2_accumulate;
    int fuse_bn_stats;
    int brick;
    int defer_head_pg;
    int persistent_deep;
    int guard;
    int reserved[3];
} dreg_exec_opts;
void dreg_exec_default_opts(dreg_exec_opts* o);
void* dreg_exec_create_opts(const int* tensors, int nt, const int* ops, int nops, const int64_t* params, int np, const dreg_exec_opts* opts);
#define DREG_EGUARD (-3)
int dreg_exec_guard_bands(void* h);
int dreg_exec_guard_check(void* h, void* arena, long long* out4, void* stream);
int dreg_exec_guard_describe(void* h, int band, char* buf, int buf_bytes);
int dreg_exec_guard_last(void* h, int* op, int* pass, long long* band);
void dreg_exec_destroy(void* h);
size_t dreg_exec_arena_bytes(void* h);
size_t dreg_exec_pack_bytes(void* h);
int dreg_exec_num_packs(void* h);
size_t dreg_exec_tensor_offset(void* h, int slot);
int dreg_exec_output_slot(void* h);
int dreg_exec_pack_rows(void* h);
int dreg_exec_export_pack_table(void* h, void* host_out, int* host_row_desc, void* pack_base);
int dreg_exec_repack(void* h, const void* descs_dev, const int* row_desc_dev, void* stream);
int dreg_exec_op_halo(void* h, int op);
void dreg_exec_set_overlap(void* h, int enable);
void dreg_exec_set_input_row_occupancy(void* h, const uint8_t* rowocc);
void dreg_exec_set_timing(void* h, int enable);
int dreg_exec_read_timings(void* h, int* op_kind, float* ms, int max);
int dreg_exec_forward(void* h, void* arena, size_t arena_bytes, const void* pack_base, const void* x_in,
                      const int64_t* rowlists, int nlists, int train, void* stream);
int dreg_exec_backward(void* h, void* arena, size_t arena_bytes, const void* pack_base, const void* x_in,
                       const void* grad_out, const int64_t* rowlists, int nlists, void* stream, void* aux_stream);
int dreg_exec_backward_range(void* h, void* arena, size_t arena_bytes, const void* pack_base, const void* x_in, const void* grad_out,
                             const int64_t* rowlists, int nlists, void* stream, void* aux_stream, int op_begin, int op_end, int flags);

int dreg_mha_fwd(const void* q, const void* k, const void* v, void* o, float* lse, int Nq, int Nk, int H,
                 int ldq, int ldk, int ldv, int ldo, float scale, int dtype, void* stream);
int dreg_mha_bwd(const void* q, const void* k, const void* v, const void* o, const void* dout, const float* lse,
                 float* dvec, void* dq, void* dk, void* dv, int Nq, int Nk, int H,
                 int ldq, int ldk, int ldv, int ldo, float scale, int dtype, void* stream);
int dreg_corr_attention_fwd(const void* q, const void* k, const float* xyz, float* out, float* lse, int L, int Nq, int Nk,
                            float scale, int dtype, void* stream);
int dreg_corr_attention_bwd(const void* q, const void* k, const float* xyz, const float* out, const float* dout,
                            const float* lse, float* dvec, void* dq, void* dk, int L, int Nq, int Nk,
                            float scale, int dtype, void* stream);

int dreg_mha_varlen_fwd(const void* q, const void* k, const void* v, void* o, float* lse, const int* probs, int nprob,
                        int max_q, int max_k, int R, int H, int ldq, int ldk, int ldv, int ldo, float scale, int dtype, void* stream);
int dreg_mha_varlen_bwd(const void* q, const void* k, const void* v, const void* o, const void* dout, const float* lse,
                        float* dvec, void* dq, void* dk, void* dv, const int* probs, int nprob, int max_q, int max_k, int R, int H,
                        int ldq, int ldk, int ldv, int ldo, float scale, int dtype, void* stream);
int dreg_corr_attention_varlen_fwd(const void* q, const void* k, const float* xyz, float* out, float* lse, const int* probs, int nprob,
                                   int max_q, int max_k, int L, int R, float scale, int dtype, void* stream);
int dreg_corr_attention_varlen_bwd(const void* q, const void* k, const float* xyz, const float* out, const float* dout,
                                   const float* lse, float* dvec, void* dq, void* dk, const int* probs, int nprob,
                                   int max_q, int max_k, int L, int R, float scale, int dtype, void* stream);

int dreg_layernorm_fwd(const float* x, const float* gamma, const float* beta, const float* pe, void* y, float* stats,
                       int N, int C, float eps, int out_dtype, void* stream);
size_t dreg_layernorm_bwd_workspace_bytes(int N);
int dreg_layernorm_bwd(const float* x, const void* dy, const float* gamma, const float* stats, float* dx, float* dgamma,
                       float* dbeta, float* workspace, int N, int C, int g_dtype, int accumulate_dx, int accumulate_w,
                       void* stream);
int dreg_layernorm_bwd_add(const float* x, const void* dy, const float* gamma, const float* stats, float* dx, const float* dx_add, float* dgamma,
                           float* dbeta, float* workspace, int N, int C, int g_dtype, int accumulate_w, void* stream);

int dreg_layernorm_fwd2(const float* x, const float* gamma, const float* beta, const float* pe, int pe_rows, float* y32, void* y16, float* stats,
                        int N, int C, float eps, void* stream);
int dreg_layernorm_bwd_parts(const float* x, const void* dy, const void* dy2_bf16, const float* gamma, const float* stats, float* dx, const float* dx_add,
                             const float* dx_add2, void* dx_bf16, float* part, int N, int C, int g_dtype, void* stream);
int dreg_layernorm_bwd_blocks(int N);
int dreg_layernorm_bwd_final_batched(const void* descs_dev, int n, void* stream);

int dreg_posenc_sine(const float* xyz, float* pe, int N, float scale, float temperature, void* stream);

int dreg_overlap_fwd(const float* f, const float* w, const float* b, float* s, int N, void* stream);
size_t dreg_overlap_bwd_workspace_bytes(int N);
int dreg_overlap_bwd(const float* f, const float* w, const float* s, const float* gy, float* df, float* dw, float* db,
                     float* workspace, int N, void* stream);

int dreg_overlap_bwd_acc(const float* f, const float* w, const float* s, const float* gy, float* df, const float* df_add, float* dw, float* db,
                         int accumulate_w, float* workspace, int N, void* stream);

int dreg_relu_bwd(const void* y, const void* g, void* out, size_t n, int y_dtype, int g_dtype, int out_dtype, void* stream);

int dreg_weighted_kabsch(const float* a, const float* b, const float* w, float* out, int P, int N, float eps, void* stream);
int dreg_weighted_kabsch_pairs(const float* xyz, const float* corr, const float* ov, const int* probs, float* out, int P, int L,
                               int R, float eps, void* stream);
int dreg_weighted_kabsch_bwd(const float* a, const float* b, const float* w, const float* g_out, float* g_a, float* g_b, float* g_w, int P, int N,
                             float eps, void* stream);
int dreg_weighted_kabsch_pairs_bwd(const float* xyz, const float* corr, const float* ov, const int* probs, const float* g_out, float* g_corr,
                                   float* g_ov, int P, int L, int R, float eps, void* stream);

int dreg_reg_point_losses(const float* gt, const float* tilde, const float* ov, const float* corr, const float* xyz,
                          const float* pose, const int* probs, float* partial, float* d_ov, float* d_corr, int L, int R, int P,
                          int robust, float eps, float w_overlap, float w_corr, void* stream);
int dreg_gemm_f32_desc_bytes(void);
int dreg_gemm_f32_batched(const void* descs_dev, int n, int total_tiles, const float* const* bases8, void* stream);
int dreg_infonce_wsym(const float* W, float* out, int E, void* stream);
int dreg_infonce_nn(const float* xyz, const float* pose, const int* probs, const int* src_off, int* nn, float* mask,
                    float* count, int P, int total_src, float r_p, void* stream);
int dreg_infonce_rows(float* logits, const float* xyz, const float* pose, const int* probs, const int* src_off,
                      const long long* logit_off, const int* nn, const float* mask, const float* count, float* loss_row, int P,
                      int total_src, float r_n, float scale, int write_grad, void* stream);
int dreg_reg_losses_final(const float* partial, const float* loss_row, const float* count, const int* probs, const int* src_off,
                          float* out, int P, int L, float eps, float w_overlap, float w_cont, float w_feat, float w_corr,
                          void* stream);
int dreg_nerf_cont_deferred(const float* gt, const float* tilde, const int* probs, float* partial, float* out, int P, int L, int R,
                            float w_overlap, float w_cont, float w_feat, float w_corr, void* stream);

int dreg_halfspace_labels(const float* xyz, const float* corr, float* gt, float* tilde, int L, int R, void* stream);

size_t dreg_voxel_downsample_workspace_bytes(int N);
int dreg_voxel_downsample_fwd(const float* pts, const float* feats, const int* pt_batch, float* out_pts, float* out_feats,
                              int* n_out, int* batch_counts, uint32_t* inv_seg, float* inv_cnt, int* err,
                              void* workspace, size_t workspace_bytes, int N, int C, int nbatch, float dl, void* stream);
int dreg_voxel_downsample_plan(const float* pts, const int* pt_batch, float* out_pts, int* n_out, int* batch_counts,
                               uint32_t* inv_seg, float* inv_cnt, int* err, uint32_t* order, uint32_t* starts,
                               void* workspace, size_t workspace_bytes, int N, int nbatch, float dl, void* stream);
int dreg_voxel_downsample_plan_frozen(const float* pts, const int* pt_batch, float* out_pts, int* n_out, int* batch_counts,
                                      uint32_t* inv_seg, float* inv_cnt, int* err, uint32_t* order, uint32_t* starts,
                                      void* workspace, size_t workspace_bytes, int N, int nbatch, float dl, const uint8_t* frozen, void* stream);
int dreg_voxel_segment_mean(const float* feats, const uint32_t* order, const uint32_t* starts, const int* n_out,
                            float* out_feats, int M, int C, void* stream);
int dreg_voxel_downsample_bwd(const float* gout, const uint32_t* inv_seg, const float* inv_cnt, float* gin, int N, int C,
                              void* stream);

int dreg_grad_norm(const float* g, float* norm_out, float* workspace, size_t n, void* stream);
int dreg_adamw_step(float* p, float* g, float* m, float* v, const float* norm, size_t n, float lr, float beta1, float beta2,
                    float eps, float weight_decay, int step, float max_norm, void* stream);

uint32_t dreg_ngp_level_table(float per_level_scale, int log2_hashmap_size, int base_resolution,
                              uint32_t* offset, uint32_t* size, uint32_t* res, float* scale, uint32_t* hashed);
int dreg_f32_to_f16(const float* in, void* out, size_t n, void* stream);
int dreg_ngp_density_fwd(const float* x, const void* table, const void* w1, const void* w2, float* density, void* raw,
                         const uint32_t* offset, const uint32_t* size, const uint32_t* res, const float* scale,
                         const uint32_t* hashed, const float* aabb, int Np, void* stream);
int dreg_ngp_dir_bias(const float* dirs, const void* w1_f16, float* out, int K, void* stream);
int dreg_ngp_alpha_keep(const float* density, float* alpha, uint8_t* keep, int N, float delta, float threshold, void* stream);
int dreg_ngp_rgb_mean_fwd(const void* raw, const void* w1, const void* w2, const void* w3, const float* dirbias, float* rgb,
                          int ndir, int Np, void* stream);
int dreg_ngp_density_fwd_contract(const float* x, const void* table, const void* w1, const void* w2, float* density, void* raw,
                                  const uint32_t* offset, const uint32_t* size, const uint32_t* res, const float* scale, const uint32_t* hashed,
                                  const float* aabb, int Np, int contract, void* stream);
size_t dreg_ngp_density_workspace_bytes(int Np);
int dreg_ngp_density_fwd_ws(const float* x, const void* table, const void* w1, const void* w2, float* density, void* raw,
                            const uint32_t* offset, const uint32_t* size, const uint32_t* res, const float* scale, const uint32_t* hashed,
                            const float* aabb, int Np, int contract, void* workspace, size_t workspace_bytes, const int* order, int x_in_slot_order, void* stream);
int dreg_grid_sample_points_ordered(const int64_t* idx, const float* jitter, const int* order, float* world, float* world_slot,
                                    int rx, int ry, int rz, const float* aabb, int Np, void* stream);
size_t dreg_grid_x_order_workspace_bytes(int rx, int ry, int rz);
int dreg_grid_x_order(const uint8_t* binary, const int64_t* idx, int* order, void* workspace, size_t workspace_bytes, int rx, int ry, int rz, int Np, void* stream);
size_t dreg_grid_occupied_workspace_bytes(int rx, int ry, int rz);
void* dreg_grid_occupied_totals(void* workspace, int rx, int ry, int rz);
int dreg_grid_occupied_count(const uint8_t* binary, void* workspace, size_t workspace_bytes, int rx, int ry, int rz, void* stream);
int dreg_grid_occupied_build(const uint8_t* binary, void* workspace, const float* jitter, const float* aabb, int64_t* indices, int* order,
                             float* world, float* world_slot, int rx, int ry, int rz, int N, void* stream);
int dreg_ngp_density_keep_fwd_ws(const float* x, const void* table, const void* w1, const void* w2, float* density, void* raw,
                                 const uint32_t* offset, const uint32_t* size, const uint32_t* res, const float* scale, const uint32_t* hashed,
                                 const float* aabb, int Np, int contract, void* workspace, size_t workspace_bytes, const int* order, int x_in_slot_order,
                                 float* alpha, uint8_t* keep, float delta, float threshold, void* stream);
int dreg_grid_write_kept(void* occ_workspace, const float* xyz, const float* rgb, const float* alpha, const int64_t* indices, const uint8_t* keep,
                         int64_t* mask, float* grid, int rx, int ry, int rz, int Np, void* stream);
int dreg_ngp_rgb_dir_fwd(const void* raw, const void* w1, const void* w2, const void* w3, const float* dirs, float* rgb, int Np, void* stream);
int dreg_grid_sample_points(const int64_t* idx, const float* jitter, float* world, int rx, int ry, int rz, const float* aabb,
                            int Np, void* stream);
int dreg_grid_scatter7(const float* xyz, const float* rgb, const float* alpha, const int64_t* idx, const uint8_t* keep,
                       float* grid, int Np, void* stream);

int dreg_surface_visibility(const float* cams, const float* pts, const uint8_t* binary, int* label,
                            const void* table, const void* w1, const void* w2,
                            const uint32_t* offset, const uint32_t* size, const uint32_t* res, const float* scale,
                            const uint32_t* hashed, const float* roi_aabb, const float* scene_aabb, const float* model_aabb,
                            int rx, int ry, int rz, int Nc, int Np, float render_step_size, float cut_off, float early_stop_eps,
                            float alpha_thre, void* stream);
int dreg_surface_visibility_queue(const float* cams, const float* pts, const uint8_t* binary, int* label,
                                  const void* table, const void* w1, const void* w2,
                                  const uint32_t* offset, const uint32_t* size, const uint32_t* res, const float* scale, const uint32_t* hashed,
                                  const float* roi_aabb, const float* scene_aabb, const float* model_aabb,
                                  int rx, int ry, int rz, int Nc, int Np, float render_step_size, float cut_off, float early_stop_eps,
                                  float alpha_thre, void* queue, const uint32_t* coarse_bits, void* stream);
int dreg_occupancy_coarse_bits(const uint8_t* binary, uint32_t* bits, int rx, int ry, int rz, void* stream);
size_t dreg_surface_visibility_desc_bytes(void);
int dreg_surface_visibility_fill_desc(void* host_desc, const float* cams, const float* pts, const uint8_t* binary, int* label,
                                      const void* table, const void* w1, const void* w2,
                                      const uint32_t* offset, const uint32_t* size, const uint32_t* res, const float* scale, const uint32_t* hashed,
                                      const float* roi_aabb, const float* scene_aabb, const float* model_aabb,
                                      int rx, int ry, int rz, int Nc, int Np, float render_step_size, float cut_off, float early_stop_eps,
                                      float alpha_thre, void* queue, const uint32_t* coarse_bits);
int dreg_surface_visibility_multi(const void* descs_dev, int n, long total_rays, void* stream);
int dreg_surface_visibility_multi_waves(const void* descs_dev, int n, long total_rays, int max_waves, void* stream);

int dreg_ngp_render(const float* origins, const float* viewdirs, long n_rays, const uint8_t* binary, int rx, int ry, int rz, const uint32_t* coarse_bits,
                    const void* table, const void* w1, const void* w2, const void* cw1, const void* cw2, const void* cw3,
                    const uint32_t* offset, const uint32_t* size, const uint32_t* res, const float* scale, const uint32_t* hashed,
                    const float* roi_aabb, const float* scene_aabb, const float* model_aabb, float near_plane, float far_plane,
                    float render_step_size, float alpha_thre, float early_stop_eps, const float* bkgd,
                    float* rgb, float* opacity, float* depth, unsigned long long* n_samples, void* queue, void* stream);

int dreg_ngp_render_pair(long n_rays,
                         const float* src_origins, const float* src_viewdirs, const uint8_t* src_binary, int src_rx, int src_ry, int src_rz,
                         const uint32_t* src_coarse_bits, const void* src_table, const void* src_w1, const void* src_w2,
                         const void* src_cw1, const void* src_cw2, const void* src_cw3,
                         const uint32_t* src_offset, const uint32_t* src_size, const uint32_t* src_res, const float* src_scale, const uint32_t* src_hashed,
                         const float* src_roi_aabb, const float* src_scene_aabb, const float* src_model_aabb,
                         float src_near_plane, float src_far_plane, float src_render_step_size, float src_alpha_thre, const float* src_center,
                         const float* tgt_origins, const float* tgt_viewdirs, const uint8_t* tgt_binary, int tgt_rx, int tgt_ry, int tgt_rz,
                         const uint32_t* tgt_coarse_bits, const void* tgt_table, const void* tgt_w1, const void* tgt_w2,
                         const void* tgt_cw1, const void* tgt_cw2, const void* tgt_cw3,
                         const uint32_t* tgt_offset, const uint32_t* tgt_size, const uint32_t* tgt_res, const float* tgt_scale, const uint32_t* tgt_hashed,
                         const float* tgt_roi_aabb, const float* tgt_scene_aabb, const float* tgt_model_aabb,
                         float tgt_near_plane, float tgt_far_plane, float tgt_render_step_size, float tgt_alpha_thre, const float* tgt_center,
                         float power, float early_stop_eps, const float* bkgd,
                         float* rgb, float* opacity, float* depth, float* weight_src, unsigned long long* n_samples, void* queue, void* stream);

int dreg_ngp_render_train(const float* origins, const float* viewdirs, const float* jitter, long n_rays, const uint8_t* binary, int rx, int ry, int rz,
                          const uint32_t* coarse_bits, const void* table, const void* w1, const void* w2, const void* cw1, const void* cw2, const void* cw3,
                          const uint32_t* offset, const uint32_t* size, const uint32_t* res, const float* scale, const uint32_t* hashed,
                          const float* roi_aabb, const float* scene_aabb, const float* model_aabb, float near_plane, float far_plane,
                          float render_step_size, float alpha_thre, float early_stop_eps, const float* bkgd,
                          float* rgb, float* opacity, float* depth, unsigned long long* n_samples, void* queue, void* stream);
size_t dreg_ngp_render_bwd_workspace_bytes(long n_rays);
int dreg_ngp_render_bwd(const float* origins, const float* viewdirs, const float* jitter, long n_rays, const uint8_t* binary, int rx, int ry, int rz,
                        const uint32_t* coarse_bits, const void* base16, const void* color16,
                        const uint32_t* offset, const uint32_t* size, const uint32_t* res, const float* scale, const uint32_t* hashed,
                        const float* roi_aabb, const float* scene_aabb, const float* model_aabb, float near_plane, float far_plane,
                        float render_step_size, float alpha_thre, float early_stop_eps,
                        const float* rgb, const float* grad_rgb, float* grad_base, float* grad_color, void* workspace, size_t workspace_bytes, void* stream);
int dreg_ngp_adam_step(float* p, float* g, float* m, float* v, void* p16, size_t n, float lr, float beta1, float beta2, float eps, int step, void* stream);

size_t dreg_image_metrics_workspace_bytes(int N, int H, int W, int C);
int dreg_image_metrics(const float* pred, const float* gt, int N, int H, int W, int C, const float* taps, float* ssim, float* mse, float* psnr,
                       float* ssim_map, uint8_t* pred_u8, uint8_t* gt_u8, void* workspace, size_t workspace_bytes, void* stream);

int dreg_ngp_density_grad(const float* x, const void* table, const void* w1, const void* w2, float* density, float* grad, unsigned long long* relu_mask,
                          const uint32_t* offset, const uint32_t* size, const uint32_t* res, const float* scale, const uint32_t* hashed,
                          const float* aabb, int Np, int contract, void* stream);

size_t dreg_icp_workspace_bytes(int Ns, int iters);
int dreg_icp_refine(const float* src, int Ns, const float* tgt_points, const float* tgt_normals, const int* perm, const int* cell_start, int Nt,
                    const float* grid_lo, float cell, int nx, int ny, int nz, double* pose, float max_dist, int iters,
                    double tol_rot, double tol_trans, double eps_cond, double* stats, double* sums, int* corr, float* dist2,
                    void* workspace, size_t workspace_bytes, void* stream);

size_t dreg_pose_ransac_workspace_bytes(int N, int H);
int dreg_pose_ransac(const float* a, const float* b, int N, const int* triplets, int H, float thresh, float eps_area, void* workspace,
                     size_t workspace_bytes, int* best, float* pose, int* status, int* counts, float* poses, unsigned char* mask, void* stream);
int dreg_pose_inliers(const float* a, const float* b, int N, const float* pose, float thresh, unsigned char* mask, int* count, void* stream);

int dreg_mc_table(signed char* tris, int* width);
size_t dreg_mc_workspace_bytes(int nx, int ny, int nz);
int dreg_mc_count(const float* values, int nx, int ny, int nz, float level, void* workspace, size_t workspace_bytes, int* counts, void* stream);
int dreg_mc_emit(const float* values, int nx, int ny, int nz, float level, const float* origin, const float* spacing, const void* workspace,
                 size_t workspace_bytes, float* verts, int* faces, int V, int F, void* stream);

int dreg_brick_supported(int B, int D, int H, int W, int Cin, int Cout);
size_t dreg_conv3_brick_pack_bytes(int rows, int red);
int dreg_pack_conv_weight_brick(const float* w, void* out, int Cout, int Cin, int transposed, void* stream);
size_t dreg_brick_tiles_workspace_bytes(int B, int D, int H, int W);
int dreg_brick_tiles_build(const uint8_t* flags, int B, int D, int H, int W, int max_rows, int max_tiles, void* workspace, size_t workspace_bytes,
                           int* meta, int* rows_sorted, void* tiles, int* halo_vox, void* nbr, void* stream);
int dreg_conv3_brick(const void* in, const void* wpk, void* out, const float* bias, const void* addend, const void* tiles, int ntiles,
                     const int* halo_vox, const void* nbr, const int* rows_sorted,
                     int B, int D, int H, int W, int Cin, int Cout, int Da, int Ha, int Wa, int add_same, int out_f32, void* stream);

int dreg_ps_num_params(void);
int dreg_ps_num_linears(void);
void* dreg_ps_create(const int64_t* params);
void dreg_ps_destroy(void* h);
void dreg_ps_set_fuse(void* h, int fuse);
void dreg_ps_set_group_wgrad(void* h, int on);
void dreg_ps_set_timing(void* h, int enable);
int dreg_ps_read_timings(void* h, int* info, float* ms, int cap);
size_t dreg_ps_arena_bytes(void* h, int R);
int dreg_ps_forward(void* h, void* arena, size_t arena_bytes, const int64_t* packs, const float* feats, const float* xyz, const float* pe,
                    const int* probs_self, const int* probs_cross, int nprob, int max_len, int R,
                    float* cond, float* corr, float* ov, void* stream);
int dreg_ps_backward(void* h, void* arena, size_t arena_bytes, const int64_t* packs, const float* feats, const float* xyz, const float* pe,
                     const int* probs_self, const int* probs_cross, int nprob, int max_len, int R,
                     const float* cond, const float* corr, const float* ov, const float* g_cond, const float* g_corr, const float* g_ov,
                     float* d_feats, void* stream, void* aux_stream, int last_only);

#ifdef __cplusplus
}
#endif
#endif
```

Measured before the change: 257.4 pairs/s.

## Fuse linear, residual, layernorm and next linear into panel kernels

```diff
diff --git a/dreg_nerf_amd/csrc/common.h b/dreg_nerf_amd/csrc/common.h
--- a/dreg_nerf_amd/csrc/common.h
+++ b/dreg_nerf_amd/csrc/common.h
@@ -49,6 +49,59 @@
     return v;
 }
 
+template <int N>
+__device__ __forceinline__ void wave_sum_n(float (&v)[N]) {
+#pragma unroll
+    for (int o = 32; o > 0; o >>= 1) {
+        float w[N];
+#pragma unroll
+        for (int n = 0; n < N; ++n) w[n] = __shfl_xor(v[n], o, 64);
+#pragma unroll
+        for (int n = 0; n < N; ++n) v[n] += w[n];
+    }
+}
+
+template <int N>
+__device__ __forceinline__ void ln_rows_fwd(const float4 (&v)[N], const float4 g, const float4 b, float eps, float (&o)[N][4], float (&mean)[N], float (&rstd)[N]) {
+#pragma unroll
+    for (int n = 0; n < N; ++n) mean[n] = v[n].x + v[n].y + v[n].z + v[n].w;
+    wave_sum_n(mean);
+    float d[N][4], var[N];
+#pragma unroll
+    for (int n = 0; n < N; ++n) {
+        mean[n] = mean[n] * (1.f / 256.f);
+        d[n][0] = v[n].x - mean[n]; d[n][1] = v[n].y - mean[n]; d[n][2] = v[n].z - mean[n]; d[n][3] = v[n].w - mean[n];
+        var[n] = d[n][0] * d[n][0] + d[n][1] * d[n][1] + d[n][2] * d[n][2] + d[n][3] * d[n][3];
+    }
+    wave_sum_n(var);
+#pragma unroll
+    for (int n = 0; n < N; ++n) {
+        rstd[n] = 1.0f / sqrtf(var[n] * (1.f / 256.f) + eps);
+        o[n][0] = d[n][0] * rstd[n] * g.x + b.x; o[n][1] = d[n][1] * rstd[n] * g.y + b.y; o[n][2] = d[n][2] * rstd[n] * g.z + b.z; o[n][3] = d[n][3] * rstd[n] * g.w + b.w;
+    }
+}
+
+template <int N>
+__device__ __forceinline__ void ln_rows_bwd(const float4 (&v)[N], const float (&d)[N][4], const float (&mean)[N], const float (&rstd)[N], const float (&gv)[4],
+                                            float (&xh)[N][4], float (&o)[N][4]) {
+    float s1[N], s2[N];
+#pragma unroll
+    for (int n = 0; n < N; ++n) {
+        xh[n][0] = (v[n].x - mean[n]) * rstd[n]; xh[n][1] = (v[n].y - mean[n]) * rstd[n]; xh[n][2] = (v[n].z - mean[n]) * rstd[n]; xh[n][3] = (v[n].w - mean[n]) * rstd[n];
+        s1[n] = 0.f; s2[n] = 0.f;
+#pragma unroll
+        for (int i = 0; i < 4; ++i) { s1[n] += d[n][i] * gv[i]; s2[n] += d[n][i] * gv[i] * xh[n][i]; }
+    }
+    wave_sum_n(s1);
+    wave_sum_n(s2);
+#pragma unroll
+    for (int n = 0; n < N; ++n) {
+        s1[n] = s1[n] * (1.f / 256.f); s2[n] = s2[n] * (1.f / 256.f);
+#pragma unroll
+        for (int i = 0; i < 4; ++i) o[n][i] = rstd[n] * (d[n][i] * gv[i] - s1[n] - xh[n][i] * s2[n]);
+    }
+}
+
 #ifdef DREG_PROBE
 #define DREG_KNOB(type, name, value) static type name = value
 #else
diff --git a/dreg_nerf_amd/csrc/pointset.hip b/dreg_nerf_amd/csrc/pointset.hip
--- a/dreg_nerf_amd/csrc/pointset.hip
+++ b/dreg_nerf_amd/csrc/pointset.hip
@@ -17,12 +17,12 @@
     const int row = blockIdx.x * 4 + (threadIdx.x >> 6), lane = threadIdx.x & 63;
     if (row >= N) return;
     const float4 v = *reinterpret_cast<const float4*>(x + (size_t)row * 256 + lane * 4);
-    const float mean = wave_sum(v.x + v.y + v.z + v.w) * (1.f / 256.f);
-    const float d0 = v.x - mean, d1 = v.y - mean, d2 = v.z - mean, d3 = v.w - mean;
-    const float var = wave_sum(d0 * d0 + d1 * d1 + d2 * d2 + d3 * d3) * (1.f / 256.f);
-    const float rstd = 1.0f / sqrtf(var + eps);
     const float4 gg = *reinterpret_cast<const float4*>(g + lane * 4), bb = *reinterpret_cast<const float4*>(b + lane * 4);
-    float o[4] = {d0 * rstd * gg.x + bb.x, d1 * rstd * gg.y + bb.y, d2 * rstd * gg.z + bb.z, d3 * rstd * gg.w + bb.w};
+    const float4 v1[1] = {v};
+    float o1[1][4], mean1[1], rstd1[1];
+    ln_rows_fwd<1>(v1, gg, bb, eps, o1, mean1, rstd1);
+    float (&o)[4] = o1[0];
+    const float mean = mean1[0], rstd = rstd1[0];
     if (pe) { const float4 p = *reinterpret_cast<const float4*>(pe + (size_t)row * 256 + lane * 4); o[0] += p.x; o[1] += p.y; o[2] += p.z; o[3] += p.w; }
     st4(y + (size_t)row * 256 + lane * 4, o);
     if (lane == 0) { stats[2 * row] = mean; stats[2 * row + 1] = rstd; }
@@ -79,14 +79,13 @@
         for (int u = 0; u < U; ++u) {
             const int row = rb + 4 * u;
             if (row < rend) {
-                const float xh[4] = {(v[u].x - mean[u]) * rstd[u], (v[u].y - mean[u]) * rstd[u], (v[u].z - mean[u]) * rstd[u], (v[u].w - mean[u]) * rstd[u]};
-                float s1 = 0.f, s2 = 0.f;
-#pragma unroll
-                for (int i = 0; i < 4; ++i) { s1 += d[u][i] * gv[i]; s2 += d[u][i] * gv[i] * xh[i]; dg[i] += d[u][i] * xh[i]; db[i] += d[u][i]; }
-                s1 = wave_sum(s1) * (1.f / 256.f); s2 = wave_sum(s2) * (1.f / 256.f);
-                float o[4];
-#pragma unroll
-                for (int i = 0; i < 4; ++i) o[i] = rstd[u] * (d[u][i] * gv[i] - s1 - xh[i] * s2);
+                const float4 v1[1] = {v[u]};
+                const float d1[1][4] = {{d[u][0], d[u][1], d[u][2], d[u][3]}}, m1[1] = {mean[u]}, r1[1] = {rstd[u]};
+                float xh[1][4], o1[1][4];
+                ln_rows_bwd<1>(v1, d1, m1, r1, gv, xh, o1);
+#pragma unroll
+                for (int i = 0; i < 4; ++i) { dg[i] += d[u][i] * xh[0][i]; db[i] += d[u][i]; }
+                float (&o)[4] = o1[0];
                 if (dx_add) { o[0] += old[u].x; o[1] += old[u].y; o[2] += old[u].z; o[3] += old[u].w; }
                 if (dx_add2) { o[0] += old2[u].x; o[1] += old2[u].y; o[2] += old2[u].z; o[3] += old2[u].w; }
                 *reinterpret_cast<float4*>(dx + (size_t)row * 256 + lane * 4) = make_float4(o[0], o[1], o[2], o[3]);
diff --git a/dreg_nerf_amd/csrc/pointset_exec.hip b/dreg_nerf_amd/csrc/pointset_exec.hip
--- a/dreg_nerf_amd/csrc/pointset_exec.hip
+++ b/dreg_nerf_amd/csrc/pointset_exec.hip
@@ -46,6 +46,7 @@
     Lin lin[NLIN];
     Layout lay;
     int fuse = 1;
+    int panel = 2;
     int group_wgrad = 1;
     std::vector<hipEvent_t> ev;
     hipEvent_t ev_done = nullptr;
@@ -190,7 +191,7 @@
     if (p->pinned) (void)hipHostFree(p->pinned);
     delete p;
 }
-void dreg_ps_set_fuse(void* h, int fuse) { ((Ps*)h)->fuse = fuse ? 1 : 0; }
+void dreg_ps_set_fuse(void* h, int fuse) { ((Ps*)h)->fuse = fuse ? 1 : 0; ((Ps*)h)->panel = fuse >= 3 ? 2 : fuse >= 2 ? 1 : 0; }
 void dreg_ps_set_group_wgrad(void* h, int on) { ((Ps*)h)->group_wgrad = on ? 1 : 0; }
 void dreg_ps_set_timing(void* h, int enable) { ((Ps*)h)->timing = enable != 0; }
 int dreg_ps_read_timings(void* h, int* info, float* ms, int cap)
@@ -222,23 +223,48 @@
     const float sc = 0.17677669529663687f;
     auto pk = [&](int li, int t) { return (const void*)packs[2 * li + t]; };
     const float* xin = feats;
+    const bool panel = p->fuse && p->panel;
+    auto chain = [&](const void* a1, int li1, int b1, const float* res, float* x, int nw, int nb, const float* pe_, void* hh, float* stt, int li2, int b2,
+                     void* out2, int k1, int n2, int relu) {
+        PsScope sc(p, stream, 3, R, k1, n2, 0);
+        return dreg_ps_panel_fwd(a1, pk(li1, 0), p->val[b1], res, x, p->val[nw], p->val[nb], pe_, hh, stt, pk(li2, 0), p->val[b2], out2, R, k1, n2, relu, 1e-5f, stream);
+    };
     for (int l = 0; l < NL; ++l) {
         const LayerBuf& b = y.L[l];
         const int o = l * PL_COUNT;
         float* xout = (float*)(A + y.allx) + (size_t)l * R * E;
-        CK(dreg_layernorm_fwd(xin, p->val[o + N1W], p->val[o + N1B], pe, A + b.h1, (float*)(A + b.st1), R, E, 1e-5f, 0, stream));
-        CK(linear_fwd(p, y, A, A + b.h1, pk(lin_index(l, LIN_SI), 0), p->val[o + SIB], nullptr, A + b.qkv1, R, E, E3, 0, 0, stream));
+        if (l == 0 || !panel) {
+            CK(dreg_layernorm_fwd(xin, p->val[o + N1W], p->val[o + N1B], pe, A + b.h1, (float*)(A + b.st1), R, E, 1e-5f, 0, stream));
+            CK(linear_fwd(p, y, A, A + b.h1, pk(lin_index(l, LIN_SI), 0), p->val[o + SIB], nullptr, A + b.qkv1, R, E, E3, 0, 0, stream));
+        }
         CK(dreg_mha_varlen_fwd(A + b.qkv1, A + b.qkv1 + E * 2, A + b.qkv1 + 2 * E * 2, A + b.o1, (float*)(A + b.lse1), probs_self, nprob, max_len, max_len,
                                R, NH, E3, E3, E3, E, sc, 0, stream));
-        CK(linear_fwd(p, y, A, A + b.o1, pk(lin_index(l, LIN_SO), 0), p->val[o + SOB], xin, A + b.xa, R, E, E, 0, 1, stream));
-        CK(dreg_layernorm_fwd((const float*)(A + b.xa), p->val[o + N2W], p->val[o + N2B], pe, A + b.h2, (float*)(A + b.st2), R, E, 1e-5f, 0, stream));
-        CK(linear_fwd(p, y, A, A + b.h2, pk(lin_index(l, LIN_CI), 0), p->val[o + CIB], nullptr, A + b.qkv2, R, E, E3, 0, 0, stream));
+        if (panel) {
+            CK(chain(A + b.o1, lin_index(l, LIN_SO), o + SOB, xin, (float*)(A + b.xa), o + N2W, o + N2B, pe, A + b.h2, (float*)(A + b.st2),
+                     lin_index(l, LIN_CI), o + CIB, A + b.qkv2, E, E3, 0));
+        } else {
+            CK(linear_fwd(p, y, A, A + b.o1, pk(lin_index(l, LIN_SO), 0), p->val[o + SOB], xin, A + b.xa, R, E, E, 0, 1, stream));
+            CK(dreg_layernorm_fwd((const float*)(A + b.xa), p->val[o + N2W], p->val[o + N2B], pe, A + b.h2, (float*)(A + b.st2), R, E, 1e-5f, 0, stream));
+            CK(linear_fwd(p, y, A, A + b.h2, pk(lin_index(l, LIN_CI), 0), p->val[o + CIB], nullptr, A + b.qkv2, R, E, E3, 0, 0, stream));
+        }
         CK(dreg_mha_varlen_fwd(A + b.qkv2, A + b.qkv2 + E * 2, A + b.qkv2 + 2 * E * 2, A + b.o2, (float*)(A + b.lse2), probs_cross, nprob, max_len, max_len,
                                R, NH, E3, E3, E3, E, sc, 0, stream));
-        CK(linear_fwd(p, y, A, A + b.o2, pk(lin_index(l, LIN_CO), 0), p->val[o + COB], A + b.xa, A + b.xb, R, E, E, 0, 1, stream));
-        CK(dreg_layernorm_fwd((const float*)(A + b.xb), p->val[o + N3W], p->val[o + N3B], nullptr, A + b.h3, (float*)(A + b.st3), R, E, 1e-5f, 0, stream));
-        CK(linear_fwd(p, y, A, A + b.h3, pk(lin_index(l, LIN_1), 0), p->val[o + L1B], nullptr, A + b.f, R, E, FF, 1, 0, stream));
-        CK(linear_fwd(p, y, A, A + b.f, pk(lin_index(l, LIN_2), 0), p->val[o + L2B], A + b.xb, xout, R, FF, E, 0, 1, stream));
+        if (panel) {
+            CK(chain(A + b.o2, lin_index(l, LIN_CO), o + COB, (const float*)(A + b.xa), (float*)(A + b.xb), o + N3W, o + N3B, nullptr, A + b.h3, (float*)(A + b.st3),
+                     lin_index(l, LIN_1), o + L1B, A + b.f, E, FF, 1));
+        } else {
+            CK(linear_fwd(p, y, A, A + b.o2, pk(lin_index(l, LIN_CO), 0), p->val[o + COB], A + b.xa, A + b.xb, R, E, E, 0, 1, stream));
+            CK(dreg_layernorm_fwd((const float*)(A + b.xb), p->val[o + N3W], p->val[o + N3B], nullptr, A + b.h3, (float*)(A + b.st3), R, E, 1e-5f, 0, stream));
+            CK(linear_fwd(p, y, A, A + b.h3, pk(lin_index(l, LIN_1), 0), p->val[o + L1B], nullptr, A + b.f, R, E, FF, 1, 0, stream));
+        }
+        if (panel && l + 1 < NL) {
+            const LayerBuf& nb = y.L[l + 1];
+            const int no = o + PL_COUNT;
+            CK(chain(A + b.f, lin_index(l, LIN_2), o + L2B, (const float*)(A + b.xb), xout, no + N1W, no + N1B, pe, A + nb.h1, (float*)(A + nb.st1),
+                     lin_index(l + 1, LIN_SI), no + SIB, A + nb.qkv1, FF, E3, 0));
+        } else {
+            CK(linear_fwd(p, y, A, A + b.f, pk(lin_index(l, LIN_2), 0), p->val[o + L2B], A + b.xb, xout, R, FF, E, 0, 1, stream));
+        }
         xin = xout;
     }
     const int R6 = NL * R;
@@ -283,6 +309,12 @@
     struct GroupRec { char d[160]; int variant, nblocks; };
     std::vector<GroupRec> grp;
     const bool group = fuse && p->group_wgrad && !p->timing;
+    const bool panel = fuse && p->panel >= 2;
+    auto panel_bwd = [&](const void* g1, const void* w1t, const float* x, const float* stt, const float* gamma, const float* add, const float* add2, float* dx, void* dx_bf,
+                         float* part, const void* w2t, void* out2, int k1, int n2) {
+        PsScope sc(p, stream, 4, R, k1, n2, 0);
+        return dreg_ps_panel_bwd(g1, w1t, x, stt, gamma, add, add2, dx, dx_bf, part, w2t, out2, R, k1, n2, stream);
+    };
     auto param_grads = [&](int li, const void* g, const void* x, int rows, size_t wg_off, size_t cs_off) -> int {
         const Lin& l = p->lin[li];
         bool grouped = false;
@@ -373,29 +405,49 @@
             CK(dreg_relu_bwd(A + b.f, A + y.dO, A + b.gF, (size_t)R * FF, 0, 0, 0, stream));
         }
         CK(param_grads(lin_index(l, LIN_2), Gbf, A + b.f, R, b.wg[LIN_2], b.cs[LIN_2]));
+        float* Gb = (float*)(A + y.gx[0]);
+        if (panel) {
+            CK(panel_bwd(A + b.gF, pk(lin_index(l, LIN_1), 1), (const float*)(A + b.xb), (const float*)(A + b.st3), p->val[o + N3W], G, nullptr, Gb, A + b.gB,
+                                 (float*)(A + b.lnp[2]), pk(lin_index(l, LIN_CO), 1), A + y.dO, FF, E));
+            CK(param_grads(lin_index(l, LIN_1), A + b.gF, A + b.h3, R, b.wg[LIN_1], b.cs[LIN_1]));
+            ln_rec(b.lnp[2], o + N3W, o + N3B, R);
+        } else {
         CK(linear_dgrad(p, y, A, A + b.gF, pk(lin_index(l, LIN_1), 1), A + y.dH, nullptr, nullptr, R, E, FF, stream));
         CK(param_grads(lin_index(l, LIN_1), A + b.gF, A + b.h3, R, b.wg[LIN_1], b.cs[LIN_1]));
-        float* Gb = (float*)(A + y.gx[0]);
         CK(dreg_layernorm_bwd_parts((const float*)(A + b.xb), A + y.dH, nullptr, p->val[o + N3W], (const float*)(A + b.st3), Gb, G, nullptr, A + b.gB,
                                     (float*)(A + b.lnp[2]), R, E, 0, stream));
         ln_rec(b.lnp[2], o + N3W, o + N3B, R);
         CK(linear_dgrad(p, y, A, A + b.gB, pk(lin_index(l, LIN_CO), 1), A + y.dO, nullptr, nullptr, R, E, E, stream));
+        }
         CK(param_grads(lin_index(l, LIN_CO), A + b.gB, A + b.o2, R, b.wg[LIN_CO], b.cs[LIN_CO]));
         CK(dreg_mha_varlen_bwd(A + b.qkv2, A + b.qkv2 + E * 2, A + b.qkv2 + 2 * E * 2, A + b.o2, A + y.dO, (const float*)(A + b.lse2), (float*)(A + y.dvec),
                                A + b.gQ2, A + b.gQ2 + E * 2, A + b.gQ2 + 2 * E * 2, probs_cross, nprob, max_len, max_len, R, NH, E3, E3, E3, E, sc, 0, stream));
+        float* Ga = (float*)(A + y.gx[1]);
+        if (panel) {
+            CK(panel_bwd(A + b.gQ2, pk(lin_index(l, LIN_CI), 1), (const float*)(A + b.xa), (const float*)(A + b.st2), p->val[o + N2W], Gb, nullptr, Ga, A + b.gC,
+                                 (float*)(A + b.lnp[1]), pk(lin_index(l, LIN_SO), 1), A + y.dO, E3, E));
+            CK(param_grads(lin_index(l, LIN_CI), A + b.gQ2, A + b.h2, R, b.wg[LIN_CI], b.cs[LIN_CI]));
+            ln_rec(b.lnp[1], o + N2W, o + N2B, R);
+        } else {
         CK(linear_dgrad(p, y, A, A + b.gQ2, pk(lin_index(l, LIN_CI), 1), A + y.dH, nullptr, nullptr, R, E, E3, stream));
         CK(param_grads(lin_index(l, LIN_CI), A + b.gQ2, A + b.h2, R, b.wg[LIN_CI], b.cs[LIN_CI]));
-        float* Ga = (float*)(A + y.gx[1]);
         CK(dreg_layernorm_bwd_parts((const float*)(A + b.xa), A + y.dH, nullptr, p->val[o + N2W], (const float*)(A + b.st2), Ga, Gb, nullptr, A + b.gC,
                                     (float*)(A + b.lnp[1]), R, E, 0, stream));
         ln_rec(b.lnp[1], o + N2W, o + N2B, R);
         CK(linear_dgrad(p, y, A, A + b.gC, pk(lin_index(l, LIN_SO), 1), A + y.dO, nullptr, nullptr, R, E, E, stream));
+        }
         CK(param_grads(lin_index(l, LIN_SO), A + b.gC, A + b.o1, R, b.wg[LIN_SO], b.cs[LIN_SO]));
         CK(dreg_mha_varlen_bwd(A + b.qkv1, A + b.qkv1 + E * 2, A + b.qkv1 + 2 * E * 2, A + b.o1, A + y.dO, (const float*)(A + b.lse1), (float*)(A + y.dvec),
                                A + b.gQ1, A + b.gQ1 + E * 2, A + b.gQ1 + 2 * E * 2, probs_self, nprob, max_len, max_len, R, NH, E3, E3, E3, E, sc, 0, stream));
-        CK(linear_dgrad(p, y, A, A + b.gQ1, pk(lin_index(l, LIN_SI), 1), A + y.dH, nullptr, nullptr, R, E, E3, stream));
+        if (!panel) CK(linear_dgrad(p, y, A, A + b.gQ1, pk(lin_index(l, LIN_SI), 1), A + y.dH, nullptr, nullptr, R, E, E3, stream));
         CK(param_grads(lin_index(l, LIN_SI), A + b.gQ1, A + b.h1, R, b.wg[LIN_SI], b.cs[LIN_SI]));
-        if (l == 0) {
+        if (panel) {
+            float* Gprev = l == 0 ? d_feats : dallx + (size_t)(l - 1) * R * E;
+            void* Gprev_bf = l == 0 ? nullptr : A + y.dallx_bf + (size_t)(l - 1) * R * E * 2;
+            CK(panel_bwd(A + b.gQ1, pk(lin_index(l, LIN_SI), 1), xin, (const float*)(A + b.st1), p->val[o + N1W], Ga, (l == 0 || last_only) ? nullptr : Gprev, Gprev,
+                                 Gprev_bf, (float*)(A + b.lnp[0]), nullptr, nullptr, E3, 0));
+            if (l > 0) { G = Gprev; Gbf = Gprev_bf; }
+        } else if (l == 0) {
             CK(dreg_layernorm_bwd_parts(xin, A + y.dH, nullptr, p->val[o + N1W], (const float*)(A + b.st1), d_feats, Ga, nullptr, nullptr,
                                         (float*)(A + b.lnp[0]), R, E, 0, stream));
         } else {
diff --git a/dreg_nerf_amd/csrc/pointset_panel.hip b/dreg_nerf_amd/csrc/pointset_panel.hip
--- /dev/null
+++ b/dreg_nerf_amd/csrc/pointset_panel.hip
@@ -0,0 +1,326 @@
+#include "common.h"
+#include "../../include/dreg_nerf.h"
+
+namespace {
+
+constexpr int PM = 64;
+constexpr int PC = 256;
+constexpr int PNW = 8;
+constexpr int W_BYTES = PC * 128, A_BYTES = PM * 128, STG = W_BYTES + A_BYTES;
+constexpr int H_OFF = 64 * 1024, P0_OFF = 96 * 1024, B2_OFF = 128 * 1024, MAX_N2 = 1024, PANEL_LDS = B2_OFF + MAX_N2 * 4;
+static_assert(3 * STG <= B2_OFF && PM * PC * 4 <= H_OFF && H_OFF + PM * PC * 2 <= P0_OFF && P0_OFF + W_BYTES <= B2_OFF && PANEL_LDS <= 160 * 1024, "LDS plan");
+
+struct PanelArgs {
+    const bf16_t* a1; const bf16_t* w1; const bf16_t* w2; bf16_t* out2;
+    int R, K1, N2, relu;
+    float eps;
+    const float* gamma;
+    const float* bias1; const float* residual; float* xout; const float* beta; const float* pe; bf16_t* hout; float* stats; const float* bias2;
+    const float* x; const float* st; const float* dx_add; const float* dx_add2; float* dx; bf16_t* dx_bf; float* part;
+};
+
+__device__ __forceinline__ void wg_barrier() {
+    asm volatile("s_waitcnt lgkmcnt(0)" ::: "memory");
+    __builtin_amdgcn_s_barrier();
+    asm volatile("" ::: "memory");
+}
+
+__device__ __forceinline__ uint32_t pswz(int row, int slot) { return (uint32_t)row * 128u + (uint32_t)((slot ^ ((row >> 1) & 7)) << 4); }
+
+template <bool BWD>
+__global__ __launch_bounds__(PNW * 64) void ps_panel_kernel(const PanelArgs a)
+{
+    typedef __attribute__((address_space(3))) void* lds_ptr_t;
+    constexpr uint32_t OOB = 0x7fffff00u;
+    extern __shared__ __attribute__((aligned(16))) char smem[];
+    const int t = threadIdx.x, lane = t & 63;
+    const int wave = __builtin_amdgcn_readfirstlane(t >> 6);
+    const int m0 = blockIdx.x * PM;
+    const int fr = lane & 15, kg = lane >> 4;
+    const int R = a.R, K1 = a.K1, N2 = a.N2;
+
+    const __amdgpu_buffer_rsrc_t rs_a = __builtin_amdgcn_make_buffer_rsrc((void*)a.a1, 0, (uint32_t)R * (uint32_t)(K1 * 2), 0x00020000);
+    const __amdgpu_buffer_rsrc_t rs_w1 = __builtin_amdgcn_make_buffer_rsrc((void*)a.w1, 0, (uint32_t)(PC * K1 * 2), 0x00020000);
+    const __amdgpu_buffer_rsrc_t rs_o2 = __builtin_amdgcn_make_buffer_rsrc((void*)a.out2, 0, (uint32_t)R * (uint32_t)(N2 * 2), 0x00020000);
+    const __amdgpu_buffer_rsrc_t rs_w2 = __builtin_amdgcn_make_buffer_rsrc((void*)a.w2, 0, (uint32_t)(N2 * PC * 2), 0x00020000);
+
+    uint32_t wrow[4], wgl[4];
+#pragma unroll
+    for (int i = 0; i < 4; ++i) {
+        const int r = (wave * 4 + i) * 8 + (lane >> 3);
+        wrow[i] = (uint32_t)r;
+        wgl[i] = (uint32_t)(((lane & 7) ^ ((r >> 1) & 7)) * 16);
+    }
+    uint32_t avoff;
+    {
+        const int r = wave * 8 + (lane >> 3);
+        const int gl = (lane & 7) ^ ((r >> 1) & 7);
+        avoff = (m0 + r < R) ? (uint32_t)(m0 + r) * (uint32_t)(K1 * 2) + (uint32_t)(gl * 16) : OOB;
+    }
+
+    constexpr int RPW = PM / PNW;
+    auto row_of = [&](int q) -> int { return BWD ? (wave >> 1) * 16 + (wave & 1) * 2 + (q >> 2) + 4 * (q & 3) : wave * RPW + q; };
+    float4 r0[RPW], r1[RPW], r2[RPW];
+    float mean_[RPW], rstd_[RPW];
+#pragma unroll
+    for (int q = 0; q < RPW; ++q) {
+        const int row = m0 + row_of(q);
+        r0[q] = make_float4(0.f, 0.f, 0.f, 0.f); r1[q] = r0[q]; r2[q] = r0[q]; mean_[q] = 0.f; rstd_[q] = 0.f;
+        if (row < R) {
+            const size_t o = (size_t)row * PC + lane * 4;
+            if constexpr (BWD) {
+                r0[q] = *reinterpret_cast<const float4*>(a.x + o);
+                if (a.dx_add) r1[q] = *reinterpret_cast<const float4*>(a.dx_add + o);
+                if (a.dx_add2) r2[q] = *reinterpret_cast<const float4*>(a.dx_add2 + o);
+                mean_[q] = a.st[2 * row]; rstd_[q] = a.st[2 * row + 1];
+            } else {
+                r0[q] = *reinterpret_cast<const float4*>(a.residual + o);
+                if (a.pe) r1[q] = *reinterpret_cast<const float4*>(a.pe + o);
+            }
+        }
+    }
+
+    const float4 gg = *reinterpret_cast<const float4*>(a.gamma + lane * 4);
+    float4 b1 = make_float4(0.f, 0.f, 0.f, 0.f), bb = b1, b2v = b1;
+    if constexpr (!BWD) {
+        b1 = *reinterpret_cast<const float4*>(a.bias1 + lane * 4); bb = *reinterpret_cast<const float4*>(a.beta + lane * 4);
+        if (t * 4 < N2) b2v = *reinterpret_cast<const float4*>(a.bias2 + t * 4);
+    }
+
+    f32x4_t acc[4][2];
+    auto zero_acc = [&]() {
+#pragma unroll
+        for (int i = 0; i < 4; ++i)
+#pragma unroll
+            for (int j = 0; j < 2; ++j) acc[i][j] = (f32x4_t){0.f, 0.f, 0.f, 0.f};
+    };
+
+    {
+        const int nk = K1 >> 6;
+        auto issue = [&](int k, int buf) {
+            char* sW = smem + buf * STG + wave * 4096;
+            char* sA = smem + buf * STG + W_BYTES + wave * 1024;
+            const uint32_t so = (uint32_t)(k * 128);
+#pragma unroll
+            for (int i = 0; i < 4; ++i)
+                __builtin_amdgcn_raw_ptr_buffer_load_lds(rs_w1, (lds_ptr_t)(sW + i * 1024), 16, (int)(wrow[i] * (uint32_t)(K1 * 2) + wgl[i]), (int)so, 0, 0);
+            __builtin_amdgcn_raw_ptr_buffer_load_lds(rs_a, (lds_ptr_t)sA, 16, (int)avoff, (int)so, 0, 0);
+        };
+        zero_acc();
+        for (int s = 0; s < 2 && s < nk; ++s) issue(s, s);
+        int cbuf = 0, ibuf = 2;
+        for (int k = 0; k < nk; ++k) {
+            if (k + 1 < nk) asm volatile("s_waitcnt vmcnt(5)" ::: "memory"); else asm volatile("s_waitcnt vmcnt(0)" ::: "memory");
+            wg_barrier();
+            if (k + 2 < nk) issue(k + 2, ibuf);
+            const char* sW = smem + cbuf * STG;
+            const char* sA = sW + W_BYTES;
+#pragma unroll
+            for (int ks = 0; ks < 2; ++ks) {
+                bf16x8_t af[4], bf[2];
+#pragma unroll
+                for (int i = 0; i < 4; ++i) af[i] = *reinterpret_cast<const bf16x8_t*>(sA + pswz(i * 16 + fr, ks * 4 + kg));
+#pragma unroll
+                for (int j = 0; j < 2; ++j) bf[j] = *reinterpret_cast<const bf16x8_t*>(sW + pswz(wave * 32 + j * 16 + fr, ks * 4 + kg));
+#pragma unroll
+                for (int i = 0; i < 4; ++i)
+#pragma unroll
+                    for (int j = 0; j < 2; ++j)
+                        acc[i][j] = __builtin_amdgcn_mfma_f32_16x16x32_bf16(bf[j], af[i], acc[i][j], 0, 0, 0);
+            }
+            cbuf = cbuf == 2 ? 0 : cbuf + 1;
+            ibuf = ibuf == 2 ? 0 : ibuf + 1;
+        }
+    }
+    float* sC = reinterpret_cast<float*>(smem);
+    wg_barrier();
+    if constexpr (!BWD) { if (t * 4 < N2) *reinterpret_cast<float4*>(smem + B2_OFF + t * 16) = b2v; }
+#pragma unroll
+    for (int i = 0; i < 4; ++i) {
+        const int row = i * 16 + fr;
+#pragma unroll
+        for (int j = 0; j < 2; ++j) {
+            const int gr = ((wave * 32 + j * 16) >> 2) + kg;
+            *reinterpret_cast<f32x4_t*>(sC + row * PC + ((gr ^ fr) << 2)) = acc[i][j];
+        }
+    }
+    const int nst = (N2 >> 8) * 4;
+    auto slot2 = [&](int s) -> char* { const int m = s & 3; return smem + (m == 0 ? P0_OFF : m == 3 ? H_OFF : (m - 1) * W_BYTES); };
+    auto issue2 = [&](int s) {
+        char* sW = slot2(s) + wave * 4096;
+        const uint32_t so = (uint32_t)((s >> 2) * (PC * PC * 2) + (s & 3) * 128);
+#pragma unroll
+        for (int i = 0; i < 4; ++i)
+            __builtin_amdgcn_raw_ptr_buffer_load_lds(rs_w2, (lds_ptr_t)(sW + i * 1024), 16, (int)(wrow[i] * (uint32_t)(PC * 2) + wgl[i]), (int)so, 0, 0);
+    };
+    if constexpr (!BWD) { if (nst > 0) issue2(0); }
+    wg_barrier();
+
+    auto put_h = [&](int lrow, uint2 hb) { *reinterpret_cast<uint2*>(smem + H_OFF + (lane >> 4) * A_BYTES + pswz(lrow, (lane & 15) >> 1) + (lane & 1) * 8) = hb; };
+    float4 cv[RPW];
+#pragma unroll
+    for (int q = 0; q < RPW; ++q) { const int lrow = row_of(q); cv[q] = *reinterpret_cast<const float4*>(sC + lrow * PC + ((lane ^ (lrow & 15)) << 2)); }
+    if constexpr (!BWD) {
+#pragma unroll
+        for (int q = 0; q < RPW; ++q) {
+            cv[q].x += b1.x; cv[q].y += b1.y; cv[q].z += b1.z; cv[q].w += b1.w;
+            cv[q].x += r0[q].x; cv[q].y += r0[q].y; cv[q].z += r0[q].z; cv[q].w += r0[q].w;
+        }
+        float o[RPW][4], mean[RPW], rstd[RPW];
+        ln_rows_fwd<RPW>(cv, gg, bb, a.eps, o, mean, rstd);
+#pragma unroll
+        for (int q = 0; q < RPW; ++q) {
+            const int lrow = row_of(q), row = m0 + lrow;
+            if (a.pe) { o[q][0] += r1[q].x; o[q][1] += r1[q].y; o[q][2] += r1[q].z; o[q][3] += r1[q].w; }
+            const uint2 hb = make_uint2(f2bf2(o[q][0], o[q][1]), f2bf2(o[q][2], o[q][3]));
+            put_h(lrow, hb);
+            if (row < R) {
+                *reinterpret_cast<float4*>(a.xout + (size_t)row * PC + lane * 4) = cv[q];
+                *reinterpret_cast<uint2*>(a.hout + (size_t)row * PC + lane * 4) = hb;
+                if (lane == 0) { a.stats[2 * row] = mean[q]; a.stats[2 * row + 1] = rstd[q]; }
+            }
+        }
+    } else {
+        const float gv[4] = {gg.x, gg.y, gg.z, gg.w};
+        float* red = reinterpret_cast<float*>(smem + P0_OFF);
+        float d[RPW][4], xh[RPW][4], o[RPW][4];
+#pragma unroll
+        for (int q = 0; q < RPW; ++q) {
+            const uint32_t w0 = f2bf2(cv[q].x, cv[q].y), w1 = f2bf2(cv[q].z, cv[q].w);
+            d[q][0] = __uint_as_float(w0 << 16); d[q][1] = __uint_as_float(w0 & 0xffff0000u); d[q][2] = __uint_as_float(w1 << 16); d[q][3] = __uint_as_float(w1 & 0xffff0000u);
+        }
+        ln_rows_bwd<RPW>(r0, d, mean_, rstd_, gv, xh, o);
+#pragma unroll
+        for (int vv = 0; vv < 2; ++vv) {
+            float dg[4] = {0.f, 0.f, 0.f, 0.f}, db[4] = {0.f, 0.f, 0.f, 0.f};
+#pragma unroll
+            for (int u = 0; u < 4; ++u) {
+                const int q = vv * 4 + u;
+                const int lrow = row_of(q), row = m0 + lrow;
+                const bool valid = row < R;
+#pragma unroll
+                for (int i = 0; i < 4; ++i) { dg[i] = valid ? dg[i] + d[q][i] * xh[q][i] : dg[i]; db[i] = valid ? db[i] + d[q][i] : db[i]; }
+                if (a.dx_add) { o[q][0] += r1[q].x; o[q][1] += r1[q].y; o[q][2] += r1[q].z; o[q][3] += r1[q].w; }
+                if (a.dx_add2) { o[q][0] += r2[q].x; o[q][1] += r2[q].y; o[q][2] += r2[q].z; o[q][3] += r2[q].w; }
+                const uint2 hb = make_uint2(f2bf2(o[q][0], o[q][1]), f2bf2(o[q][2], o[q][3]));
+                put_h(lrow, hb);
+                if (valid) {
+                    *reinterpret_cast<float4*>(a.dx + (size_t)row * PC + lane * 4) = make_float4(o[q][0], o[q][1], o[q][2], o[q][3]);
+                    if (a.dx_bf) *reinterpret_cast<uint2*>(a.dx_bf + (size_t)row * PC + lane * 4) = hb;
+                }
+            }
+            float* rw = red + ((wave >> 1) * 4 + (wave & 1) * 2 + vv) * 512;
+#pragma unroll
+            for (int i = 0; i < 4; ++i) { rw[lane * 4 + i] = dg[i]; rw[256 + lane * 4 + i] = db[i]; }
+        }
+        wg_barrier();
+#pragma unroll
+        for (int b = 0; b < 4; ++b) {
+            if (m0 + b * 16 >= R) break;
+            const float* rb = red + b * 4 * 512 + t;
+            a.part[(size_t)((m0 >> 4) + b) * 512 + t] = rb[0] + rb[512] + rb[1024] + rb[1536];
+        }
+    }
+    wg_barrier();
+    if (nst == 0) return;
+
+    if constexpr (BWD) issue2(0);
+    issue2(1);
+    issue2(2);
+    bf16x8_t ah[8][4];
+#pragma unroll
+    for (int kk = 0; kk < 8; ++kk)
+#pragma unroll
+        for (int i = 0; i < 4; ++i) ah[kk][i] = *reinterpret_cast<const bf16x8_t*>(smem + H_OFF + (kk >> 1) * A_BYTES + pswz(i * 16 + fr, (kk & 1) * 4 + kg));
+    zero_acc();
+    for (int c = 0; c < (N2 >> 8); ++c) {
+#pragma unroll
+        for (int kc = 0; kc < 4; ++kc) {
+            const int s = c * 4 + kc;
+            {
+                const bool last = c + 1 == (N2 >> 8);
+                const int n = (kc < 2 ? 8 : kc == 2 ? (last ? 4 : 8) : (last ? 0 : 8)) + ((c > 0 && kc < 3) ? 8 : 0);
+                if (n == 0) asm volatile("s_waitcnt vmcnt(0)" ::: "memory");
+                else if (n == 4) asm volatile("s_waitcnt vmcnt(4)" ::: "memory");
+                else if (n == 8) asm volatile("s_waitcnt vmcnt(8)" ::: "memory");
+                else if (n == 12) asm volatile("s_waitcnt vmcnt(12)" ::: "memory");
+                else asm volatile("s_waitcnt vmcnt(16)" ::: "memory");
+            }
+            wg_barrier();
+            if (s + 3 < nst) issue2(s + 3);
+            const char* sW = slot2(s);
+#pragma unroll
+            for (int ks = 0; ks < 2; ++ks) {
+                bf16x8_t bf[2];
+#pragma unroll
+                for (int j = 0; j < 2; ++j) bf[j] = *reinterpret_cast<const bf16x8_t*>(sW + pswz(wave * 32 + j * 16 + fr, ks * 4 + kg));
+#pragma unroll
+                for (int i = 0; i < 4; ++i)
+#pragma unroll
+                    for (int j = 0; j < 2; ++j)
+                        acc[i][j] = __builtin_amdgcn_mfma_f32_16x16x32_bf16(bf[j], ah[kc * 2 + ks][i], acc[i][j], 0, 0, 0);
+            }
+        }
+#pragma unroll
+        for (int j = 0; j < 2; ++j) {
+            const int n = c * PC + wave * 32 + j * 16 + kg * 4;
+            float4 b2 = make_float4(0.f, 0.f, 0.f, 0.f);
+            if constexpr (!BWD) b2 = *reinterpret_cast<const float4*>(smem + B2_OFF + n * 4);
+#pragma unroll
+            for (int i = 0; i < 4; ++i) {
+                const int row = m0 + i * 16 + fr;
+                float v[4] = {acc[i][j][0], acc[i][j][1], acc[i][j][2], acc[i][j][3]};
+                if constexpr (!BWD) {
+                    v[0] += b2.x; v[1] += b2.y; v[2] += b2.z; v[3] += b2.w;
+                    if (a.relu) {
+#pragma unroll
+                        for (int e = 0; e < 4; ++e) v[e] = fmaxf(v[e], 0.f);
+                    }
+                }
+                typedef __attribute__((ext_vector_type(2))) unsigned int u32x2_t;
+                const u32x2_t w = {f2bf2(v[0], v[1]), f2bf2(v[2], v[3])};
+                __builtin_amdgcn_raw_buffer_store_b64(w, rs_o2, (int)(((uint32_t)row * (uint32_t)N2 + (uint32_t)n) * 2u), 0, 0);
+            }
+        }
+        zero_acc();
+    }
+}
+
+template <bool BWD>
+int panel_launch(const PanelArgs& a, void* stream)
+{
+    if ((uint64_t)a.R * (uint64_t)a.K1 * 2 >= 0x7fffff00ull || (uint64_t)(a.R + PM) * (uint64_t)a.N2 * 2 >= 0x7fffff00ull || a.N2 > MAX_N2) return DREG_EINVAL;
+    static const hipError_t attr = hipFuncSetAttribute((const void*)ps_panel_kernel<BWD>, hipFuncAttributeMaxDynamicSharedMemorySize, PANEL_LDS);
+    if (attr != hipSuccess) return DREG_ELAUNCH;
+    hipLaunchKernelGGL(ps_panel_kernel<BWD>, dim3((a.R + PM - 1) / PM), dim3(PNW * 64), PANEL_LDS, (hipStream_t)stream, a);
+    DREG_LAUNCH_CHECK();
+    return DREG_OK;
+}
+
+}
+
+extern "C" int dreg_ps_panel_fwd(const void* a1, const void* w1_packed, const float* bias1, const float* residual, float* x_out,
+                                 const float* gamma, const float* beta, const float* pe, void* h_out, float* stats,
+                                 const void* w2_packed, const float* bias2, void* out2, int R, int K1, int N2, int relu, float eps, void* stream)
+{
+    if (R <= 0 || K1 <= 0 || K1 % 64 || N2 <= 0 || N2 % PC) return DREG_EINVAL;
+    if (!a1 || !w1_packed || !bias1 || !residual || !x_out || !gamma || !beta || !h_out || !stats || !w2_packed || !bias2 || !out2) return DREG_EINVAL;
+    PanelArgs a{};
+    a.a1 = (const bf16_t*)a1; a.w1 = (const bf16_t*)w1_packed; a.w2 = (const bf16_t*)w2_packed; a.out2 = (bf16_t*)out2;
+    a.R = R; a.K1 = K1; a.N2 = N2; a.relu = relu; a.eps = eps; a.gamma = gamma;
+    a.bias1 = bias1; a.residual = residual; a.xout = x_out; a.beta = beta; a.pe = pe; a.hout = (bf16_t*)h_out; a.stats = stats; a.bias2 = bias2;
+    return panel_launch<false>(a, stream);
+}
+
+extern "C" int dreg_ps_panel_bwd(const void* g1, const void* w1t_packed, const float* x, const float* stats, const float* gamma,
+                                 const float* dx_add, const float* dx_add2, float* dx, void* dx_bf16, float* part,
+                                 const void* w2t_packed, void* out2, int R, int K1, int N2, void* stream)
+{
+    if (R <= 0 || K1 <= 0 || K1 % 64 || (N2 != 0 && N2 != PC)) return DREG_EINVAL;
+    if (!g1 || !w1t_packed || !x || !stats || !gamma || !dx || !part || (N2 && (!w2t_packed || !out2))) return DREG_EINVAL;
+    PanelArgs a{};
+    a.a1 = (const bf16_t*)g1; a.w1 = (const bf16_t*)w1t_packed; a.w2 = (const bf16_t*)w2t_packed; a.out2 = (bf16_t*)out2;
+    a.R = R; a.K1 = K1; a.N2 = N2; a.gamma = gamma;
+    a.x = x; a.st = stats; a.dx_add = dx_add; a.dx_add2 = dx_add2; a.dx = dx; a.dx_bf = (bf16_t*)dx_bf16; a.part = part;
+    return panel_launch<true>(a, stream);
+}
diff --git a/dreg_nerf_amd/lib.py b/dreg_nerf_amd/lib.py
--- a/dreg_nerf_amd/lib.py
+++ b/dreg_nerf_amd/lib.py
@@ -173,6 +173,8 @@
     "dreg_ps_set_timing": (None, [P, I]),
     "dreg_ps_read_timings": (I, [P, P, P, I]),
     "dreg_ps_arena_bytes": (Z, [P, I]),
+    "dreg_ps_panel_fwd": (I, [P] * 13 + [I, I, I, I, F, P]),
+    "dreg_ps_panel_bwd": (I, [P] * 12 + [I, I, I, P]),
     "dreg_ps_forward": (I, [P, P, Z, P, P, P, P, P, P, I, I, I, P, P, P, P]),
     "dreg_ps_backward": (I, [P, P, Z, P, P, P, P, P, P, I, I, I, P, P, P, P, P, P, P, P, P, I]),
     "dreg_posenc_sine": (I, [P, P, I, F, F, P]),
diff --git a/dreg_nerf_amd/pointset_exec.py b/dreg_nerf_amd/pointset_exec.py
--- a/dreg_nerf_amd/pointset_exec.py
+++ b/dreg_nerf_amd/pointset_exec.py
@@ -19,7 +19,12 @@
             "linear1.weight", "linear2.weight")
 
 FUSE = True
+PANEL = 3
 GROUP_WGRAD = True
+
+
+def _fuse_level() -> int:
+    return 0 if not FUSE else int(PANEL)
 
 
 def param_names():
@@ -55,9 +60,9 @@
         self.h = self.lib.dreg_ps_create(tab.ctypes.data)
         if not self.h:
             raise L.DregError("dreg_ps_create failed")
-        self.lib.dreg_ps_set_fuse(self.h, int(FUSE))
+        self.lib.dreg_ps_set_fuse(self.h, _fuse_level())
         self.lib.dreg_ps_set_group_wgrad(self.h, int(GROUP_WGRAD))
-        self._fuse = FUSE
+        self._fuse = _fuse_level()
         self._group = GROUP_WGRAD
         self.device = self.params[0].device
         self.arena = None
@@ -114,7 +119,11 @@
         for i in range(n):
             kind, rows, cin, cout, flags = (info[5 * i + k] for k in range(5))
             fl = 2.0 * rows * cin * cout
-            if kind == 2:
+            if kind in (3, 4):
+                fl = 2.0 * rows * 256 * (cin + cout)
+                name = f"ps_panel_kernel<{'true' if kind == 4 else 'false'}>"
+                label = f"panel {'bwd' if kind == 4 else 'fwd'} B{rows} {cin}->256->{cout}"
+            elif kind == 2:
                 name = ops.wgrad_kernel_name(self.lib, rows, 1, 1, 1, cin, cout, 1)
                 label = f"wgrad B{rows} 1x1x1x{cin} g1x1x1x{cout} k1s1"
             elif kind == 1:
@@ -126,9 +135,9 @@
             profiler.add_measured(name, label, fl, ms[i])
 
     def forward(self, feats, xyz, pe, tab):
-        if self._fuse != FUSE:
-            self.lib.dreg_ps_set_fuse(self.h, int(FUSE))
-            self._fuse = FUSE
+        if self._fuse != _fuse_level():
+            self._fuse = _fuse_level()
+            self.lib.dreg_ps_set_fuse(self.h, self._fuse)
         if self._group != GROUP_WGRAD:
             self.lib.dreg_ps_set_group_wgrad(self.h, int(GROUP_WGRAD))
             self._group = GROUP_WGRAD
diff --git a/include/dreg_nerf.h b/include/dreg_nerf.h
--- a/include/dreg_nerf.h
+++ b/include/dreg_nerf.h
@@ -496,6 +496,12 @@
                      const int* probs_self, const int* probs_cross, int nprob, int max_len, int R,
                      const float* cond, const float* corr, const float* ov, const float* g_cond, const float* g_corr, const float* g_ov,
                      float* d_feats, void* stream, void* aux_stream, int last_only);
+int dreg_ps_panel_fwd(const void* a1, const void* w1_packed, const float* bias1, const float* residual, float* x_out,
+                      const float* gamma, const float* beta, const float* pe, void* h_out, float* stats,
+                      const void* w2_packed, const float* bias2, void* out2, int R, int K1, int N2, int relu, float eps, void* stream);
+int dreg_ps_panel_bwd(const void* g1, const void* w1t_packed, const float* x, const float* stats, const float* gamma,
+                      const float* dx_add, const float* dx_add2, float* dx, void* dx_bf16, float* part,
+                      const void* w2t_packed, void* out2, int R, int K1, int N2, void* stream);
 
 #ifdef __cplusplus
 }
```

After: 261.6 pairs/s, median of 6. 1.02x the previous value.
